# RazorClient/Stark-prover

Measured on AMD Instinct MI355X. Metric: FRI commit field-elems/sec at codeword 2^24; achieved HBM GB/s vs peak, higher is better.
Workload: dtype u32; 1 GPU; fri_commit codeword 2^24, blowup 8 (d=2^21), SHA-256 Merkle per layer, 21 rounds; codeword_log2=24, per_gpu_log2=24, blowup=8, field=p=3*2^30+1, parallelism=single GPU

## Files before the change

### stark-prover_amd/csrc/fri_commit.hip

```cpp
#include "fri_host.hpp"

void fri::plan_layout(Plan& p, size_t d, uint32_t log_n, uint32_t G, uint32_t rank, size_t& lay, size_t& tre,
                        size_t& xin) {
    const bool sharded = G > 1;
    uint32_t logG = 0;
    while ((1u << logG) < G) logG++;
    p.log_n = log_n;
    p.d = d;
    p.rmax = rounds_bound(d, log_n);
    p.sharded = sharded;
    p.G = G;
    p.rank = rank;
    p.k_sw = sharded ? switch_layer(log_n, logG, p.rmax) : -1;
    const bool local_tail = sharded && p.k_sw < p.rmax;
    p.cs0 = 0;
    if (sharded) {
        const size_t per = (d + G - 1) / G;
        while (((size_t)1 << p.cs0) < per) p.cs0++;
        if ((int)p.cs0 < p.k_sw) p.cs0 = (uint32_t)p.k_sw;
    }
    std::vector<uint32_t> block_of(G), rank_of(G);
    for (uint32_t r = 0; r < G; r++) block_of[r] = rank_of[r] = r;
    lay = tre = xin = 0;
    for (int k = 0; k <= p.rmax; k++) {
        const uint32_t L = log_n - (uint32_t)k;
        const bool blk = sharded && k <= p.k_sw;
        const uint32_t Lt = blk ? L - logG : L;
        p.layer_off[k] = lay;
        p.tree_off[k] = tre;
        p.xinv_off[k] = xin;
        p.xinv_start[k] = 0;
        p.block[k] = blk ? block_of[rank] : 0u;
        lay += (blk && !(k == p.k_sw && local_tail)) ? ((size_t)1 << Lt) : ((size_t)1 << L);
        tre += 8 * (((size_t)2 << Lt) - 1);
        if (k < p.rmax) {
            if (sharded && k < p.k_sw) {
                const size_t B = (size_t)1 << Lt;
                p.xinv_start[k] = fold_xinv_start(block_of[rank], G, B);
                xin += B / 2;
                advance_blocks(block_of, rank_of, G);
            } else {
                xin += ((size_t)1 << L) / 2;
            }
        }
    }
    p.layer_off[p.rmax + 1] = lay;
    p.tree_off[p.rmax + 1] = tre;
    p.xinv_off[p.rmax + 1] = xin;
}

int fri::plan_build(fri_ctx* ctx, size_t d, uint32_t log_n, uint32_t offset, uint32_t G, uint32_t rank) {
    Plan& p = ctx->plan;
    const bool sharded = G > 1;
    auto same = [&](const Plan& q) {
        return q.d == d && q.log_n == log_n && q.offset == offset && q.sharded == sharded && q.G == G && q.rank == rank;
    };
    if (p.valid && same(p)) return FRI_OK;
    bool stale = p.valid;
    for (const Lane& ln : ctx->lanes) stale = stale || (ln.plan.valid && !same(ln.plan));
    if (stale) plan_free(ctx);
    const size_t n = (size_t)1 << log_n;
    size_t lay, tre, xin;
    plan_layout(p, d, log_n, G, rank, lay, tre, xin);
    p.offset = offset;
    p.in_cap = d ? d : 1;
    p.coef_cap = d / 2 + 1;
    p.coefF_cap = 0;
    if (sharded) {
        const size_t S1 = p.cs0 >= 1 ? ((size_t)1 << (p.cs0 - 1)) : 1;
        const size_t Ssw = (size_t)1 << (p.cs0 - (uint32_t)p.k_sw);
        const bool local_tail = p.k_sw < p.rmax;
        p.coef_cap = std::max(S1, local_tail ? G * Ssw / 2 : (size_t)0) + 1;
        if (local_tail && p.k_sw >= 1) p.coefF_cap = G * Ssw;
    }
    const size_t nhi = log_n > POW_LO_LOG ? ((size_t)1 << (log_n - POW_LO_LOG)) : 1;
    if (dalloc(ctx, &p.d_in, p.in_cap * 4) != hipSuccess || dalloc(ctx, &p.coefA, p.coef_cap * 4) != hipSuccess ||
        dalloc(ctx, &p.coefB, p.coef_cap * 4) != hipSuccess ||
        (p.coefF_cap && dalloc(ctx, &p.coefF, p.coefF_cap * 4) != hipSuccess) ||
        dalloc(ctx, &p.layers, lay * 4) != hipSuccess ||
        dalloc(ctx, &p.trees, tre * 4) != hipSuccess || dalloc(ctx, &p.xinv, (xin ? xin : 1) * 4) != hipSuccess ||
        dalloc(ctx, &p.pre_lo, ((size_t)1 << POW_LO_LOG) * 4) != hipSuccess ||
        dalloc(ctx, &p.pre_hi, nhi * 4) != hipSuccess ||
        dalloc(ctx, &p.wgmax, 6 * ((log_n > 8 ? ((size_t)1 << (log_n - 8)) : 1) + 16) * 4) != hipSuccess) {
        plan_release(ctx, p);
        return fail(ctx, FRI_ENOMEM, "device allocation failed for commit plan");
    }
    hipStream_t s = ctx->stream;
    launch_pow_table(p.pre_lo, p.pre_hi, log_n, offset, 1u, s);
    if (sharded) {
        uint32_t offk = offset;
        for (int k = 0; k < p.rmax; k++) {
            const uint32_t L = log_n - (uint32_t)k;
            const size_t cnt = p.xinv_off[k + 1] - p.xinv_off[k];
            const uint32_t first = mul_std(offk, pow_std(root_of_unity(L), (uint64_t)p.xinv_start[k]));
            launch_coset_points(p.layers, cnt, first, L, s);
            launch_batch_inverse(p.layers, p.xinv + p.xinv_off[k], cnt, 1, s);
            offk = mul_std(offk, offk);
        }
    } else if (p.rmax > 0) {
        launch_coset_points(ctx->scratch_a, n / 2, offset, log_n, s);
        launch_batch_inverse(ctx->scratch_a, p.xinv + p.xinv_off[0], n / 2, 1, s);
        for (int k = 1; k < p.rmax; k++)
            launch_square_mont(p.xinv + p.xinv_off[k - 1], p.xinv + p.xinv_off[k], ((size_t)1 << (log_n - k)) / 2, s);
    }
    FRI_HIP(ctx, hipGetLastError());
    FRI_HIP(ctx, hipStreamSynchronize(s));
    p.valid = true;
    return FRI_OK;
}

uint32_t* fri::coef_buf(Plan& p, int r) {
    if (r == 0) return const_cast<uint32_t*>(p.src);
    return (r % 2 == 1) ? p.coefA : p.coefB;
}

LayerTask fri::commit_task(fri_ctx* ctx, int k) {
    Plan& p = ctx->plan;
    LayerTask t{};
    t.prev = k ? p.layers + p.layer_off[k - 1] : nullptr;
    t.xinv = k ? p.xinv + p.xinv_off[k - 1] : nullptr;
    t.values = p.layers + p.layer_off[k];
    t.tree = p.trees + p.tree_off[k];
    t.L = p.log_n - (uint32_t)k;
    t.k = k;
    t.coef_in = coef_buf(p, k ? k - 1 : 0);
    t.coef_out = k ? coef_buf(p, k) : nullptr;
    t.d0 = p.d;
    t.wgmax = p.wgmax;
    t.st = ctx->d_state;
    return t;
}

static void enqueue_commit(fri_ctx* ctx) {
    Plan& p = ctx->plan;
    hipStream_t s = ctx->stream;
    const uint32_t log_n = p.log_n;
    const size_t n = (size_t)1 << log_n;
    NttPlan np = lde_plan(ctx, log_n);
    np.pre_lo = p.pre_lo;
    np.pre_hi = p.pre_hi;
    np.scratch = p.trees;
    size_t sp = span_begin(ctx, "lde", p.d * 4 + n * 4);
    launch_ntt(np, p.src, p.d, p.layers + p.layer_off[0], s);
    span_end(ctx, sp);
    for (int k = 0; k <= p.rmax; k++) {
        const uint32_t L = log_n - (uint32_t)k;
        if (L <= TAIL_LOG) {
            LayerTask ts[TAIL_LOG + 1];
            uint32_t nt = 0;
            for (int kk = k; kk <= p.rmax; kk++) ts[nt++] = commit_task(ctx, kk);
            size_t spk = span_begin(ctx, k == 0 ? "layer0" : "layers", 0);
            launch_tail(ts, nt, s);
            span_end(ctx, spk);
            break;
        }
        const LayerTask t = commit_task(ctx, k);
        uint64_t leaf_nodes = 0;
        for (uint32_t j = 0; j <= 4 && j <= L; j++) leaf_nodes += (uint64_t)1 << (L - j);
        const uint64_t leaf_bytes = ((uint64_t)4 << L) + 4 * (uint64_t)p.d + 32 * leaf_nodes;
        size_t spl = (k == 0 && L >= 19) ? span_begin(ctx, "merkle_layer0_leaf", leaf_bytes) : (size_t)-1;
        size_t spk = span_begin(ctx, k == 0 ? "layer0" : "layers", 0);
        launch_layer(t, s, spl == (size_t)-1 ? nullptr : ctx->spans[spl].e);
        span_end(ctx, spk);
    }
}

void fri::init_state(fri_ctx* ctx, DevState* h, const fri_channel_state* chan_in, uint32_t flags,
                       const uint32_t* forced_betas) {
    ctx->h_state = h;
    ctx->res_lane = ctx->cur_lane;
    memset(h, 0, sizeof(DevState));
    ctx->commit_gen++;
    if (chan_in && chan_in->has_state) {
        for (int i = 0; i < 8; i++)
            h->chan[i] = ((uint32_t)chan_in->digest[4 * i] << 24) | ((uint32_t)chan_in->digest[4 * i + 1] << 16) |
                         ((uint32_t)chan_in->digest[4 * i + 2] << 8) | chan_in->digest[4 * i + 3];
        h->chan_has = 1;
    }
    h->deg0max = -1;
    h->final_degree = -1;
    for (int r = 0; r < MAXR; r++) { h->newmax[r] = -1; h->evenmax[r] = -1; h->oddmax[r] = -1; }
    for (int r = 0; r <= MAXR; r++) h->deg[r] = -1;
    if ((flags & FRI_FLAG_FORCE_BETAS) && forced_betas) {
        h->forced = 1;
        for (int r = 0; r < MAXR; r++) h->forced_beta[r] = forced_betas[r];
    }
}
int fri::commit_validate(fri_ctx* ctx, size_t d, uint32_t log_n, uint32_t offset, uint32_t flags,
                           const uint32_t* forced_betas) {
    if (log_n < 1 || log_n > ctx->log_n_max) return fail(ctx, FRI_EINVAL, "log_n out of range for context");
    const size_t n = (size_t)1 << log_n;
    if (d > n) return fail(ctx, FRI_EDEGREE, "more coefficients than domain points (domain would be exhausted)");
    if (offset == 0 || offset >= P) return fail(ctx, FRI_EINVAL, "offset must be a nonzero canonical element");
    if ((flags & FRI_FLAG_FORCE_BETAS) && !forced_betas) return fail(ctx, FRI_EINVAL, "forced betas missing");
    if (forced_betas && (flags & FRI_FLAG_FORCE_BETAS) && !check_canonical(forced_betas, MAXR))
        return fail(ctx, FRI_EINVAL, "forced beta not canonical");
    return FRI_OK;
}

int fri::commit_enqueue(fri_ctx* ctx, const uint32_t* host_coeffs, const uint32_t* dev_coeffs, size_t d,
                          uint32_t log_n, uint32_t offset, const fri_channel_state* chan_in, uint32_t flags,
                          const uint32_t* forced_betas, int slot) {
    int rv = commit_validate(ctx, d, log_n, offset, flags, forced_betas);
    if (rv) return rv;
    FRI_HIP(ctx, hipSetDevice(ctx->device));
    int rc = plan_build(ctx, d, log_n, offset);
    if (rc) return rc;
    Plan& p = ctx->plan;
    hipStream_t s = ctx->stream;
    ctx->sharded_layers = 0;
    DevState* hs = slot < 0 ? ctx->h_sync : ctx->h_slot[slot];
    init_state(ctx, hs, chan_in, flags, forced_betas);
    ctx->commit_log_n = log_n;
    if (dev_coeffs && d && ctx->user_in && dev_coeffs == ctx->user_in) {
        p.src = ctx->user_in;
    } else {
        if (host_coeffs && d)
            FRI_HIP(ctx, hipMemcpyAsync(p.d_in, host_coeffs, d * 4, hipMemcpyHostToDevice, s));
        else if (dev_coeffs && d && dev_coeffs != p.d_in)
            FRI_HIP(ctx, hipMemcpyAsync(p.d_in, dev_coeffs, d * 4, hipMemcpyDeviceToDevice, s));
        p.src = p.d_in;
    }
    const bool use_graph = !(flags & FRI_FLAG_NO_GRAPH) && !ctx->profiling;
    if (use_graph) {
        const int gs = slot < 0 ? FRI_MAX_INFLIGHT : slot;
        const int gv = p.src == p.d_in ? 0 : 1;
        hipGraph_t& pg = p.graph[gs][gv];
        hipGraphExec_t& px = p.exec[gs][gv];
        if (px && p.graph_src[gs][gv] != p.src) {
            FRI_HIP(ctx, hipStreamSynchronize(s));
            hipGraphExecDestroy(px);
            hipGraphDestroy(pg);
            px = nullptr;
            pg = nullptr;
        }
        if (!px) {
            FRI_HIP(ctx, hipStreamBeginCapture(s, hipStreamCaptureModeThreadLocal));
            hipError_t e1 = hipMemcpyAsync(ctx->d_state, hs, sizeof(DevState), hipMemcpyHostToDevice, s);
            if (e1 == hipSuccess) enqueue_commit(ctx);
            const hipError_t e2 =
                e1 == hipSuccess ? hipMemcpyAsync(hs, ctx->d_state, sizeof(DevState), hipMemcpyDeviceToHost, s) : e1;
            hipGraph_t g = nullptr;
            const hipError_t e3 = hipStreamEndCapture(s, &g);
            if (e2 != hipSuccess || e3 != hipSuccess) {
                if (g) hipGraphDestroy(g);
                FRI_HIP(ctx, e2);
                FRI_HIP(ctx, e3);
            }
            pg = g;
            FRI_HIP(ctx, hipGraphInstantiate(&px, g, nullptr, nullptr, 0));
            p.graph_src[gs][gv] = p.src;
        }
        FRI_HIP(ctx, hipGraphLaunch(px, s));
    } else {
        FRI_HIP(ctx, hipMemcpyAsync(ctx->d_state, hs, sizeof(DevState), hipMemcpyHostToDevice, s));
        enqueue_commit(ctx);
        FRI_HIP(ctx, hipGetLastError());
        FRI_HIP(ctx, hipMemcpyAsync(hs, ctx->d_state, sizeof(DevState), hipMemcpyDeviceToHost, s));
    }
    return FRI_OK;
}

int fri::commit_finish(fri_ctx* ctx, DevState* h, uint32_t log_n, fri_commit_result* out) {
    if (h->status) {
        h->n_layers = 0;
        return fail(ctx, (int)h->status, status_message(h->status));
    }
    memset(out, 0, sizeof *out);
    out->n_layers = h->n_layers;
    out->n_rounds = h->n_rounds;
    out->log_n = log_n;
    out->final_value = h->final_value;
    out->final_degree = h->final_degree;
    for (uint32_t k = 0; k < h->n_layers && k <= (uint32_t)MAXR; k++) digest_to_bytes(h->roots[k], out->roots[k]);
    for (uint32_t r = 0; r < h->n_rounds && r < (uint32_t)MAXR; r++) out->betas[r] = h->beta[r];
    digest_to_bytes(h->chan, out->channel_out.digest);
    out->channel_out.has_state = h->chan_has;
    ctx->err.clear();
    return FRI_OK;
}

int fri::run_commit(fri_ctx* ctx, const uint32_t* host_coeffs, const uint32_t* dev_coeffs, size_t d,
                      uint32_t log_n, uint32_t offset, const fri_channel_state* chan_in, uint32_t flags,
                      const uint32_t* forced_betas, fri_commit_result* out) {
    if (!ctx || !out) return fail(ctx, FRI_EINVAL, "null argument");
    int rc = commit_validate(ctx, d, log_n, offset, flags, forced_betas);
    if (rc) return rc;
    rc = use_lane(ctx, 0);
    if (rc) return rc;
    rc = commit_enqueue(ctx, host_coeffs, dev_coeffs, d, log_n, offset, chan_in, flags, forced_betas, -1);
    if (rc) return rc;
    FRI_HIP(ctx, hipStreamSynchronize(ctx->stream));
    ctx->async_unsettled = false;
    if (ctx->profiling) spans_collect(ctx);
    return commit_finish(ctx, ctx->h_state, log_n, out);
}

extern "C" int fri_commit(fri_ctx* ctx, const uint32_t* coeffs, size_t d, uint32_t log_n, uint32_t offset,
                          const fri_channel_state* chan_in, uint32_t flags, const uint32_t* forced_betas,
                          fri_commit_result* out) {
    if (d && !coeffs) return fail(ctx, FRI_EINVAL, "null coefficients");
    if (ctx && ctx->team_root) return team_commit(ctx, coeffs, nullptr, d, log_n, offset, chan_in, flags, forced_betas, out);
    return run_commit(ctx, coeffs, nullptr, d, log_n, offset, chan_in, flags, forced_betas, out);
}

extern "C" int fri_commit_device(fri_ctx* ctx, const uint32_t* d_coeffs, size_t d, uint32_t log_n,
                                 uint32_t offset, const fri_channel_state* chan_in, uint32_t flags,
                                 const uint32_t* forced_betas, fri_commit_result* out) {
    if (d && !d_coeffs) return fail(ctx, FRI_EINVAL, "null coefficients");
    if (ctx && ctx->team_root)
        return team_commit(ctx, nullptr, d_coeffs, d, log_n, offset, chan_in, flags, forced_betas, out);
    return run_commit(ctx, nullptr, d_coeffs, d, log_n, offset, chan_in, flags, forced_betas, out);
}
extern "C" int fri_debug_plan_layout(size_t d, uint32_t log_n, uint32_t world, uint32_t rank, uint64_t* out,
                                     size_t cap) {
    if (!out || log_n < 1 || log_n > 30 || world < 1 || world > 64 || (world & (world - 1)) || rank >= world)
        return FRI_EINVAL;
    uint32_t logG = 0;
    while ((1u << logG) < world) logG++;
    if (world > 1 && log_n < logG + 12) return FRI_EINVAL;
    if (cap < 4 + 5 * (size_t)(MAXR + 1)) return FRI_EINVAL;
    Plan p;
    size_t lay, tre, xin;
    plan_layout(p, d, log_n, world, rank, lay, tre, xin);
    out[0] = (uint64_t)p.rmax;
    out[1] = (uint64_t)(int64_t)p.k_sw;
    out[2] = 4 * (uint64_t)(lay + tre + xin);
    out[3] = p.cs0;
    for (int k = 0; k <= p.rmax; k++) {
        uint64_t* o = out + 4 + 5 * (size_t)k;
        o[0] = p.layer_off[k + 1] - p.layer_off[k];
        o[1] = p.tree_off[k + 1] - p.tree_off[k];
        o[2] = p.xinv_off[k + 1] - p.xinv_off[k];
        o[3] = p.xinv_start[k];
        o[4] = p.block[k];
    }
    return FRI_OK;
}
```

### stark-prover_amd/csrc/fri_host.hpp

```cpp
#pragma once
#include <hip/hip_runtime.h>
#include <stdio.h>
#include <string.h>
#include <algorithm>
#include <chrono>
#include <condition_variable>
#include <cstdlib>
#include <functional>
#include <map>
#include <memory>
#include <mutex>
#include <string>
#include <thread>
#include <vector>

#include <rccl/rccl.h>

#include "../../include/fri_amd.h"
#include "fri_internal.hpp"

#pragma GCC visibility push(hidden)

namespace fri {

static_assert(MAXR == FRI_MAX_ROUNDS, "round bound");

struct ProfEntry { double ms = 0; uint64_t launches = 0; uint64_t bytes = 0; };

struct Plan {
    bool valid = false;
    uint32_t log_n = 0;
    size_t d = 0;
    uint32_t offset = 0;
    int rmax = 0;
    bool sharded = false;
    uint32_t G = 1, rank = 0;
    int k_sw = -1;
    uint32_t cs0 = 0;
    uint32_t* coefF = nullptr;  size_t coefF_cap = 0;
    uint32_t* d_in = nullptr;   size_t in_cap = 0;
    const uint32_t* src = nullptr;
    uint32_t* coefA = nullptr;
    uint32_t* coefB = nullptr;  size_t coef_cap = 0;
    uint32_t* layers = nullptr; size_t layer_off[MAXR + 2] = {0};
    uint32_t* trees = nullptr;  size_t tree_off[MAXR + 2] = {0};
    uint32_t* xinv = nullptr;   size_t xinv_off[MAXR + 2] = {0};
    size_t xinv_start[MAXR + 2] = {0};
    uint32_t block[MAXR + 2] = {0};
    uint32_t* pre_lo = nullptr;
    uint32_t* pre_hi = nullptr;
    int32_t* wgmax = nullptr;
    hipGraph_t graph[FRI_MAX_INFLIGHT + 1][2] = {};
    hipGraphExec_t exec[FRI_MAX_INFLIGHT + 1][2] = {};
    const uint32_t* graph_src[FRI_MAX_INFLIGHT + 1][2] = {};
    hipGraph_t tail_graph = nullptr;
    hipGraphExec_t tail_exec = nullptr;
    const uint32_t* tail_src = nullptr;
    bool graph_profiled = false;
};

struct Lane {
    Plan plan;
    hipStream_t stream = nullptr;
    DevState* d_state = nullptr;
};

struct Team;

struct Transport {
    int rank = 0, world = 1;
    ncclComm_t comm = nullptr;
    ncclComm_t xcomm = nullptr;
    bool host = false;
    bool loop = false;
    bool peer = false;
    Team* team = nullptr;
    int64_t fail_at = -1;
    int64_t n_ops = 0;
    fri_collectives ops{};
    uint8_t* hs = nullptr;
    uint8_t* hr = nullptr;
    size_t hcap = 0;
    std::vector<fri_transport_op> log;
};

struct DistBuf {
    size_t cap = 0;
    uint32_t* cyc = nullptr;
    uint32_t* recv = nullptr;
    uint32_t* half = nullptr;
    uint32_t* half2 = nullptr;
    uint32_t* top = nullptr;
    uint32_t* pre_lo = nullptr;
    uint32_t* pre_hi = nullptr;
    size_t gcap = 0;
    uint32_t* gath = nullptr;
    uint32_t* dq = nullptr;
    uint32_t* rec = nullptr;
    ShardTop* shtop = nullptr;
    std::vector<ShardTop> shtop_h;
    std::vector<int32_t> sched_h;
};

struct PeerSlot {
    const void* send;
    void* recv;
    size_t bytes;
    uint32_t op, chan;
    int peer;
};

struct Team {
    uint32_t G = 1, logG = 0;
    int kind = FRI_TRANSPORT_PEER;
    std::vector<int> dev;
    std::vector<fri_ctx*> rk;
    bool can_pull = true;
    bool kernel_pull = true;
    std::vector<std::pair<int, int>> peer_pairs;
    std::vector<std::thread> th;
    std::mutex jm;
    std::condition_variable jcv, dcv;
    uint64_t seq = 0;
    uint32_t left = 0;
    bool quit = false;
    std::function<int(uint32_t)> job;
    std::vector<int> rc;
    std::mutex bm;
    std::condition_variable bcv;
    uint64_t bgen = 0;
    uint32_t arrived = 0;
    bool aborted = false;
    std::string why;
    std::vector<PeerSlot> slot;
    std::vector<hipEvent_t> ev_ready, ev_done;
};

struct TimedSpan { std::string cls; hipEvent_t b, e; uint64_t bytes; };
}

using namespace fri;

struct fri_ctx {
    int device = 0;
    uint32_t log_n_max = 0;
    hipStream_t stream = nullptr;
    std::string err;
    uint32_t* tw_fwd = nullptr;
    uint32_t* tw_inv = nullptr;
    uint32_t* scratch_a = nullptr;
    uint32_t* scratch_b = nullptr;
    uint32_t* scratch_c = nullptr;
    uint32_t* pow_lo = nullptr;
    uint32_t* pow_hi = nullptr;
    DevState* d_state = nullptr;
    DevState* h_state = nullptr;
    DevState* h_sync = nullptr;
    DevState* h_slot[FRI_MAX_INFLIGHT] = {};
    hipEvent_t ev_slot[FRI_MAX_INFLIGHT] = {};
    uint64_t slot_ticket[FRI_MAX_INFLIGHT] = {};
    uint32_t slot_log_n[FRI_MAX_INFLIGHT] = {};
    bool slot_pending[FRI_MAX_INFLIGHT] = {};
    bool slot_user[FRI_MAX_INFLIGHT] = {};
    uint32_t* h_in[FRI_MAX_INFLIGHT] = {};
    uint32_t* d_slot_in[FRI_MAX_INFLIGHT] = {};
    size_t h_in_cap[FRI_MAX_INFLIGHT] = {};
    hipEvent_t ev_in[FRI_MAX_INFLIGHT] = {};
    hipStream_t h2d_stream = nullptr;
    uint64_t next_ticket = 1;
    bool async_unsettled = false;
    Plan plan;
    Lane lanes[FRI_MAX_INFLIGHT];
    int cur_lane = 0;
    int res_lane = 0;
    int max_lanes = FRI_DEFAULT_LANES;
    int lanes_ok = FRI_MAX_INFLIGHT;
    int slot_lane[FRI_MAX_INFLIGHT] = {};
    uint64_t lane_ticket[FRI_MAX_INFLIGHT] = {};
    bool profiling = false;
    std::map<std::string, ProfEntry> prof;
    std::vector<TimedSpan> spans;
    std::vector<hipEvent_t> event_pool;
    size_t event_next = 0;
    Transport tp;
    DistBuf db;
    hipStream_t xstream = nullptr;
    hipEvent_t ev_vals = nullptr, ev_xchg = nullptr;
    hipStream_t cstream = nullptr;
    hipEvent_t ev_pre = nullptr, ev_coef = nullptr;
    uint32_t sharded_layers = 0;
    uint64_t commit_gen = 0;
    uint32_t commit_log_n = 0;
    uint32_t* interp_tmp = nullptr;
    size_t interp_cap = 0;
    uint32_t* dq_host = nullptr;
    uint32_t* dq_dev = nullptr;
    uint32_t* trace_tree = nullptr;
    uint32_t* trace_lde = nullptr;
    size_t trace_tree_cap = 0;
    bool trace_valid = false;
    uint32_t trace_log_t = 0, trace_log_b = 0, trace_offset = 0;
    bool stuck = false;
    bool inject_stall = false;
    uint32_t* stall_flag = nullptr;
    uint32_t* stall_flag_dev = nullptr;
    std::map<const void*, size_t> allocs;
    size_t dev_bytes = 0, dev_peak = 0;
    size_t dev_cap = 0;
    Team* team_root = nullptr;
    uint32_t* user_in = nullptr;
    size_t user_cap = 0;
    uint64_t* d_csum = nullptr;
    uint64_t* h_csum = nullptr;
};

namespace fri {

template <class T>
inline hipError_t dalloc(fri_ctx* ctx, T** p, size_t bytes) {
    void* q = nullptr;
    if (ctx->dev_cap && ctx->dev_bytes + bytes > ctx->dev_cap) { *p = nullptr; return hipErrorOutOfMemory; }
    const hipError_t e = hipMalloc(&q, bytes);
    if (e != hipSuccess) { *p = nullptr; return e; }
    *p = static_cast<T*>(q);
    ctx->allocs[q] = bytes;
    ctx->dev_bytes += bytes;
    if (ctx->dev_bytes > ctx->dev_peak) ctx->dev_peak = ctx->dev_bytes;
    return hipSuccess;
}
inline void dfree(fri_ctx* ctx, const void* p) {
    if (!p) return;
    auto it = ctx->allocs.find(p);
    if (it != ctx->allocs.end()) {
        ctx->dev_bytes -= it->second;
        ctx->allocs.erase(it);
    }
    hipFree(const_cast<void*>(p));
}

#define FRI_HIP(ctx, expr)                                                              \
    do {                                                                                \
        hipError_t _e = (expr);                                                         \
        if (_e != hipSuccess) {                                                         \
            (ctx)->err = std::string(#expr) + ": " + hipGetErrorString(_e);             \
            return FRI_EHIP;                                                            \
        }                                                                               \
    } while (0)

inline double rccl_timeout_s() {
    const char* e = getenv("FRI_RCCL_TIMEOUT_S");
    const double v = e ? atof(e) : 0.0;
    return v > 0.0 ? v : 120.0;
}
inline double seconds_since(std::chrono::steady_clock::time_point t0) {
    return std::chrono::duration<double>(std::chrono::steady_clock::now() - t0).count();
}
inline int fail(fri_ctx* ctx, int code, const std::string& msg) {
    if (ctx) ctx->err = msg;
    return code;
}

inline const char* status_message(uint32_t status) {
    return status == FRI_EINVAL ? "coefficient not canonical (>= p)"
                                : "degree exceeds the domain (reference would panic)";
}

inline bool check_canonical(const uint32_t* v, size_t n) {
    for (size_t i = 0; i < n; i += 16384) {
        const size_t e = n - i < 16384 ? n : i + 16384;
        uint32_t bad = 0;
        for (size_t j = i; j < e; j++) bad |= (uint32_t)(v[j] >= P);
        if (bad) return false;
    }
    return true;
}

inline int rounds_bound(size_t d, uint32_t log_n) {
    if (d <= 1) return 0;
    int b = 0;
    for (size_t v = d - 1; v; v >>= 1) b++;
    return b < (int)log_n ? b : (int)log_n;
}

constexpr uint32_t SHARD_MIN_LOG = 20;

inline bool next_layer_sharded(uint32_t log_n, uint32_t logG, int k, int rmax) {
    const uint32_t Lk = log_n - (uint32_t)k;
    return k < rmax && (Lk - 1) >= SHARD_MIN_LOG && (Lk - 1 - logG) >= 10;
}
inline int switch_layer(uint32_t log_n, uint32_t logG, int rmax) {
    int k = 0;
    while (next_layer_sharded(log_n, logG, k, rmax)) k++;
    return k;
}
inline void advance_blocks(std::vector<uint32_t>& block_of, std::vector<uint32_t>& rank_of, uint32_t G) {
    for (uint32_t r = 0; r < G; r++) {
        const uint32_t br = block_of[r];
        block_of[r] = br < G / 2 ? 2 * br : 2 * (br - G / 2) + 1;
    }
    for (uint32_t r = 0; r < G; r++) rank_of[block_of[r]] = r;
}
inline size_t fold_xinv_start(uint32_t b, uint32_t G, size_t B) {
    const bool isA = b < G / 2;
    return (size_t)(isA ? b : b - G / 2) * B + (isA ? 0 : B / 2);
}

inline NttPlan lde_plan(fri_ctx* ctx, uint32_t log_n) {
    NttPlan p{};
    p.log_n = log_n;
    p.tw = ctx->tw_fwd;
    return p;
}

inline int ensure_tmp(fri_ctx* ctx, size_t words) {
    if (words <= ctx->interp_cap) return FRI_OK;
    FRI_HIP(ctx, hipStreamSynchronize(ctx->stream));
    if (ctx->interp_tmp) dfree(ctx, ctx->interp_tmp);
    ctx->interp_tmp = nullptr;
    ctx->interp_cap = 0;
    if (dalloc(ctx, &ctx->interp_tmp, words * 4) != hipSuccess) return fail(ctx, FRI_ENOMEM, "partials scratch");
    ctx->interp_cap = words;
    return FRI_OK;
}
constexpr size_t TMP_KEEP_WORDS = (size_t)1 << 26;
inline void tmp_trim(fri_ctx* ctx) {
    if (ctx->interp_cap <= TMP_KEEP_WORDS) return;
    (void)hipStreamSynchronize(ctx->stream);
    dfree(ctx, ctx->interp_tmp);
    ctx->interp_tmp = nullptr;
    ctx->interp_cap = 0;
}

inline void digest_to_bytes(const uint32_t* w, uint8_t* out) {
    for (int i = 0; i < 8; i++) {
        out[4 * i] = (uint8_t)(w[i] >> 24); out[4 * i + 1] = (uint8_t)(w[i] >> 16);
        out[4 * i + 2] = (uint8_t)(w[i] >> 8); out[4 * i + 3] = (uint8_t)w[i];
    }
}

size_t span_begin(fri_ctx* ctx, const char* cls, uint64_t bytes);
void span_end(fri_ctx* ctx, size_t id);
void spans_collect(fri_ctx* ctx);

void plan_release(fri_ctx* ctx, Plan& p);
void plan_free(fri_ctx* ctx);
int use_lane(fri_ctx* ctx, int j);
void settle(fri_ctx* ctx);

void plan_layout(Plan& p, size_t d, uint32_t log_n, uint32_t G, uint32_t rank, size_t& lay, size_t& tre,
                 size_t& xin);
int plan_build(fri_ctx* ctx, size_t d, uint32_t log_n, uint32_t offset, uint32_t G = 1, uint32_t rank = 0);
uint32_t* coef_buf(Plan& p, int r);
LayerTask commit_task(fri_ctx* ctx, int k);
void init_state(fri_ctx* ctx, DevState* h, const fri_channel_state* chan_in, uint32_t flags,
                const uint32_t* forced_betas);
int commit_validate(fri_ctx* ctx, size_t d, uint32_t log_n, uint32_t offset, uint32_t flags,
                    const uint32_t* forced_betas);
int commit_enqueue(fri_ctx* ctx, const uint32_t* host_coeffs, const uint32_t* dev_coeffs, size_t d,
                   uint32_t log_n, uint32_t offset, const fri_channel_state* chan_in, uint32_t flags,
                   const uint32_t* forced_betas, int slot);
int commit_finish(fri_ctx* ctx, DevState* h, uint32_t log_n, fri_commit_result* out);
int run_commit(fri_ctx* ctx, const uint32_t* host_coeffs, const uint32_t* dev_coeffs, size_t d, uint32_t log_n,
               uint32_t offset, const fri_channel_state* chan_in, uint32_t flags, const uint32_t* forced_betas,
               fri_commit_result* out);

int dq_alloc(fri_ctx* ctx);

int input_checksum(fri_ctx* ctx, const uint32_t* d_src, size_t d, uint64_t* out);

int tp_host_stage(fri_ctx* ctx, size_t bytes);
void rccl_abort(fri_ctx* ctx);
int sync_sharded(fri_ctx* ctx, hipStream_t s);
int tp_allgather(fri_ctx* ctx, const void* dsend, void* drecv, size_t bytes, hipStream_t s);
int tp_alltoall(fri_ctx* ctx, const void* dsend, void* drecv, size_t bytes_per_peer, hipStream_t s);
int tp_sendrecv(fri_ctx* ctx, const void* dsend, void* drecv, size_t bytes, int peer, hipStream_t s, uint32_t chan);
int dist_buffers(fri_ctx* ctx, size_t M, uint32_t G, size_t gwords);

int run_commit_sharded(fri_ctx* ctx, const uint32_t* host_coeffs, const uint32_t* dev_coeffs, size_t d,
                       uint32_t log_n, uint32_t offset, const fri_channel_state* chan_in, uint32_t flags,
                       const uint32_t* forced_betas, fri_commit_result* out);
int decommit_sharded(fri_ctx* ctx, uint64_t index, uint32_t* values, size_t values_cap, uint8_t* paths,
                     size_t paths_cap, size_t* paths_len);

void team_abort(Team* T, const std::string& why);
bool team_barrier(Team* T);
int team_run(fri_ctx* root, const std::function<int(uint32_t)>& fn);
void team_destroy(fri_ctx* root);
int team_commit(fri_ctx* ctx, const uint32_t* host_coeffs, const uint32_t* dev_coeffs, size_t d, uint32_t log_n,
                uint32_t offset, const fri_channel_state* chan_in, uint32_t flags, const uint32_t* forced_betas,
                fri_commit_result* out);
int team_layer_copy(fri_ctx* ctx, uint32_t layer, uint32_t* out);
int team_tree_level_copy(fri_ctx* ctx, uint32_t layer, uint32_t level, uint32_t* w);
int team_decommit(fri_ctx* ctx, uint64_t index, uint32_t* values, size_t values_cap, uint8_t* paths,
                  size_t paths_cap, size_t* paths_len);

}

#pragma GCC visibility pop
```

### stark-prover_amd/csrc/fri_internal.hpp

```cpp
#pragma once
#include <hip/hip_runtime.h>
#include <stddef.h>
#include <stdint.h>
#include <functional>
#include "field.hpp"

namespace fri {

constexpr int MAXR = 32;
constexpr uint32_t TOP_LOG = 9;
#ifndef FRI_TAIL_LOG
#define FRI_TAIL_LOG 9
#endif
constexpr uint32_t TAIL_LOG = FRI_TAIL_LOG;
constexpr uint32_t POW_LO_LOG = 12;

struct DevState {
    uint32_t chan[8];
    uint32_t chan_has;
    uint32_t chan_pending;
    uint32_t n_layers;
    uint32_t n_rounds;
    uint32_t final_value;
    int32_t  final_degree;
    uint32_t status;
    uint32_t forced;
    int32_t  deg0max;
    uint32_t active[MAXR + 1];
    int32_t  deg[MAXR + 1];
    int32_t  newmax[MAXR];
    int32_t  evenmax[MAXR];
    int32_t  oddmax[MAXR];
    uint32_t beta[MAXR];
    uint32_t beta_mont[MAXR];
    uint32_t forced_beta[MAXR];
    uint32_t roots[MAXR + 1][8];
#ifdef FRI_STAMPS
    uint64_t stamps[MAXR + 1][64];
#endif
};

__host__ __device__ inline size_t level_offset(uint32_t L, uint32_t l) {
    return ((size_t)2 << L) - ((size_t)2 << (L - l));
}

struct NttPlan {
    uint32_t log_n;
    const uint32_t* tw;
    const uint32_t* pre_lo;
    const uint32_t* pre_hi;
    const uint32_t* post_lo;
    const uint32_t* post_hi;
    uint32_t* scratch;
};
void launch_ntt(const NttPlan& p, const uint32_t* src, size_t d, uint32_t* dst, hipStream_t s);

void launch_twiddles(uint32_t* tw, uint32_t log_max, bool inverse, hipStream_t s);
void launch_pow_table(uint32_t* lo, uint32_t* hi, uint32_t log_n, uint32_t base_std,
                      uint32_t scale_std, hipStream_t s);
void launch_batch_inverse(const uint32_t* in, uint32_t* out, size_t n, int out_mont,
                          hipStream_t s);
void launch_coset_points(uint32_t* out, size_t count, uint32_t offset, uint32_t log_n,
                         hipStream_t s);
void launch_square_mont(const uint32_t* in, uint32_t* out, size_t count, hipStream_t s);
size_t interp_tmp_words(size_t n, uint32_t log_N);
void launch_interp_weights(const uint32_t* xs, size_t n, uint32_t* acc, uint32_t* tmp, hipStream_t s);
void launch_interp_coeffs(const uint32_t* ys, uint32_t* w_to_c, size_t n, hipStream_t s);
void launch_interp_eval(const uint32_t* xs, const uint32_t* c, size_t n, uint32_t log_N, uint32_t* f, uint32_t* tmp,
                        hipStream_t s);
size_t evaluate_tmp_words(size_t d, size_t count);
void launch_evaluate(const uint32_t* coeffs, size_t d, const uint32_t* xs, size_t count, uint32_t* out,
                     uint32_t* tmp, hipStream_t s);
void launch_poly_pointwise_mul(const uint32_t* a, const uint32_t* b, uint32_t* out, size_t n, hipStream_t s);
void launch_poly_newton(const uint32_t* f, const uint32_t* g, uint32_t* out, size_t n, hipStream_t s);
constexpr size_t POLY_DIRECT_LIMIT = 4096;
void launch_poly_conv_direct(const uint32_t* lng, size_t ll, const uint32_t* sht, size_t ls, uint32_t* out,
                             size_t n_out, hipStream_t s);
void launch_poly_reverse(const uint32_t* src, size_t top, size_t cnt, uint32_t* dst, size_t n, hipStream_t s);
void launch_poly_sub(const uint32_t* a, const uint32_t* t, uint32_t* r, size_t n, hipStream_t s);
struct DecommitPlan {
    uint64_t index;
    uint32_t log_n, n_layers;
    uint64_t layer_off[MAXR + 1];
    uint64_t tree_off[MAXR + 1];
    uint32_t path_off[MAXR + 1];
    uint32_t logG;
    uint8_t shard_lb1[MAXR + 1];
    uint8_t val_block[MAXR + 1];
    uint64_t owned[MAXR + 1];
    uint64_t top_off[MAXR + 1];
};
void launch_decommit_gather(const uint32_t* layers, const uint32_t* trees, const DecommitPlan& dp, uint32_t* out,
                            hipStream_t s, const uint32_t* top = nullptr);
void launch_fold_plain(const uint32_t* in, uint32_t* out, uint32_t log_m, const uint32_t* xinv_m,
                       uint32_t beta, hipStream_t s);

constexpr uint32_t REC_WORDS = 16;
struct ShardTop {
    uint32_t* rec_out;
    const int32_t* rec_mx;
    const uint32_t* rec_c0;
    uint32_t rec_R;
    uint32_t G;
    const uint32_t* recs_in;
    int32_t sched_deg;
    uint32_t sched_on;
    uint8_t rank_of_block[64];
};

struct LayerTask {
    const uint32_t* prev;
    const uint32_t* xinv;
    uint32_t* values;
    uint32_t* tree;
    uint32_t L;
    int k;
    uint32_t beta_m;
    const uint32_t* coef_in;
    uint32_t* coef_out;
    size_t d0;
    int32_t* wgmax;
    DevState* st;
    const DevState* gst;
    int gidx;
    size_t jlo, jhi, ibase, obase;
    const ShardTop* shard;
    const uint32_t* prev2;
    uint32_t send_half;
    uint32_t wg_base;
    uint32_t wg_total;
};
void launch_layer(const LayerTask& t, hipStream_t s, hipEvent_t ev_leaf_end = nullptr,
                  const std::function<void()>& after_leaf = {}, hipEvent_t ev_before_top = nullptr,
                  const std::function<void()>& after_part1 = {});
void launch_tail(const LayerTask* ts, uint32_t n, hipStream_t s);
void launch_coef(const LayerTask& t, uint32_t G, hipStream_t s);
void launch_coset_coeffs(const uint32_t* a, size_t d, uint32_t* out, size_t M, uint32_t c_std, hipStream_t s);
void launch_decimate(const uint32_t* a, size_t d, uint32_t* ev, uint32_t* od, hipStream_t s);
void launch_radix2_block(const uint32_t* E, const uint32_t* O, const uint32_t* tlo, const uint32_t* thi,
                         uint32_t* out, size_t M, uint32_t negate, hipStream_t s);
void launch_cyclic_to_block(const uint32_t* recv, uint32_t* block, size_t B, uint32_t G, hipStream_t s);
void launch_place_blocks(const uint32_t* gath, uint32_t* layer, size_t B, uint32_t G, const uint32_t* block_of,
                         hipStream_t s);
struct PeerPull {
    const uint32_t* src[64];
    uint32_t* dst;
    size_t words;
    uint32_t n;
    uint32_t vec4;
};
void launch_peer_pull(const PeerPull& pp, hipStream_t s);
void launch_checksum(const uint32_t* v, size_t n, uint64_t* out, hipStream_t s);
void launch_replicate(const uint32_t* src, uint32_t* dst, size_t words, uint32_t G, hipStream_t s);
void launch_top(const LayerTask& t, uint32_t l, const int32_t* mx, uint32_t G, hipStream_t s);

constexpr uint32_t FIBSQ_MAX_B = 16;
struct FibsqParams {
    uint32_t log_n;
    uint32_t B;
    uint32_t offset_m;
    uint32_t w_m, winv_m;
    uint32_t glast_m, gprev_m;
    uint32_t a_last;
    uint32_t alpha_m[3];
    uint32_t zinv_m[FIBSQ_MAX_B];
};
void launch_fibsq_cp(const uint32_t* f_lde, uint32_t* out, const FibsqParams& q, hipStream_t s);
void launch_trace_gather(const uint32_t* lde, const uint32_t* tree, uint32_t L, uint64_t index, uint64_t stride,
                         uint32_t count, uint32_t* out, hipStream_t s);

}
```

### stark-prover_amd/csrc/fri_layer.hip

```cpp
#include "fri_internal.hpp"
#include "sha256_fast.hpp"
#include "sha256_quad.hpp"

namespace fri {

constexpr uint32_t INV2_M2 = 0x80000000u;

#ifdef FRI_STAMPS
#define TOP_STAMP(i)                                                                     \
    do {                                                                                 \
        if (COMMIT && threadIdx.x == 0) t.st->stamps[t.k][(i)] = __builtin_amdgcn_s_memrealtime(); \
    } while (0)
#define TOP_CLK(i)                                                                               \
    do {                                                                                           \
        if (COMMIT && threadIdx.x == 0) t.st->stamps[t.k][(i)] = __builtin_amdgcn_s_memtime();     \
    } while (0)
#define TOP_STAMP_T(i, tid_)                                                                       \
    do {                                                                                           \
        if (COMMIT && threadIdx.x == (tid_)) t.st->stamps[t.k][(i)] = __builtin_amdgcn_s_memrealtime(); \
    } while (0)
#else
#define TOP_STAMP(i) do {} while (0)
#define TOP_CLK(i) do {} while (0)
#define TOP_STAMP_T(i, tid_) do {} while (0)
#endif
#ifdef FRI_STAMPS
#define WIDE_STAMP(i)                                                                              \
    do {                                                                                           \
        if (COMMIT && blockIdx.x == 0 && threadIdx.x == 0) t.st->stamps[t.k][(i)] = __builtin_amdgcn_s_memrealtime(); \
    } while (0)
#else
#define WIDE_STAMP(i) do {} while (0)
#endif
#ifdef FRI_STAMPS
#define TAIL_STAMP_T(i, tid_, fn)                                                  \
    do {                                                                           \
        if (threadIdx.x == (tid_)) t.st->stamps[t.k][(i)] = fn();                  \
    } while (0)
#define TAIL_STAMP(i) TAIL_STAMP_T(i, 0, __builtin_amdgcn_s_memrealtime)
#define TAIL_CLK(i) TAIL_STAMP_T(i, 0, __builtin_amdgcn_s_memtime)
#else
#define TAIL_STAMP_T(i, tid_, fn) do {} while (0)
#define TAIL_STAMP(i) do {} while (0)
#define TAIL_CLK(i) do {} while (0)
#endif

__device__ __forceinline__ uint32_t fold1(uint32_t a, uint32_t b, uint32_t xinv_m, uint32_t beta_m) {
    uint32_t s = add(a, b), t = sub(a, b);
    return mmul(add(s, mmul(mmul(t, xinv_m), beta_m)), INV2_M2);
}

#ifndef FRI_CHAIN_PRIO
#define FRI_CHAIN_PRIO 3
#endif
__device__ __forceinline__ void chain_prio() {
    if (FRI_CHAIN_PRIO > 0) __builtin_amdgcn_s_setprio(FRI_CHAIN_PRIO);
}

struct Dg { uint32_t w[8]; };

__device__ __forceinline__ void dg_load(const uint32_t* p, Dg& d) {
    uint4 a = reinterpret_cast<const uint4*>(p)[0], b = reinterpret_cast<const uint4*>(p)[1];
    d.w[0] = a.x; d.w[1] = a.y; d.w[2] = a.z; d.w[3] = a.w; d.w[4] = b.x; d.w[5] = b.y; d.w[6] = b.z; d.w[7] = b.w;
}
__device__ __forceinline__ void dg_store(uint32_t* p, const Dg& d) {
    reinterpret_cast<uint4*>(p)[0] = make_uint4(d.w[0], d.w[1], d.w[2], d.w[3]);
    reinterpret_cast<uint4*>(p)[1] = make_uint4(d.w[4], d.w[5], d.w[6], d.w[7]);
}
__device__ __forceinline__ void dg_lds_load(const uint4* p, Dg& d) {
    uint4 a = p[0], b = p[1];
    d.w[0] = a.x; d.w[1] = a.y; d.w[2] = a.z; d.w[3] = a.w; d.w[4] = b.x; d.w[5] = b.y; d.w[6] = b.z; d.w[7] = b.w;
}
__device__ __forceinline__ void dg_lds_store(uint4* p, const Dg& d) {
    p[0] = make_uint4(d.w[0], d.w[1], d.w[2], d.w[3]);
    p[1] = make_uint4(d.w[4], d.w[5], d.w[6], d.w[7]);
}
__device__ __forceinline__ void hnode(const Dg& l, const Dg& r, Dg& o) { shaf::node(l.w, r.w, o.w); }
__device__ __forceinline__ void hleaf(uint32_t v, Dg& o) { shaf::leaf(v, o.w); }
__device__ __forceinline__ void cnode(const Dg& l, const Dg& r, Dg& o) { shaf::node_compact(l.w, r.w, o.w); }
__device__ __forceinline__ void cleaf(uint32_t v, Dg& o) { shaf::leaf_compact(v, o.w); }

__device__ __forceinline__ void pair_level(const uint4* A, uint4* B, uint32_t* out, uint32_t tid, uint32_t cnt,
                                           const shaq::Role& R) {
    if (tid >= max(2 * cnt, 64u)) return;
    const uint32_t q = (tid >> 1) & (cnt - 1), half = (tid & 1u) ^ 1u;
    const bool real = tid < 2 * cnt;
    Dg a, b;
    dg_lds_load(A + 4 * q, a);
    dg_lds_load(A + 4 * q + 2, b);
    uint32_t o[4];
    shaq::node(a.w, b.w, o, R);
    if (!real) return;
    const uint4 v = make_uint4(o[0], o[1], o[2], o[3]);
    B[2 * q + half] = v;
    reinterpret_cast<uint4*>(out + 8 * q)[half] = v;
}

#ifndef FRI_SCHED_PRODUCER
#define FRI_SCHED_PRODUCER 1
#endif
#ifndef FRI_SCHED_CHANNEL
#define FRI_SCHED_CHANNEL 0
#endif
struct SchedLds {
    uint32_t wk[32 * 48];
    uint32_t flag;
};
__device__ __forceinline__ void sched_init(SchedLds* sl) {
    if (FRI_SCHED_PRODUCER && threadIdx.x == 0) sl->flag = 0u;
}
__device__ __forceinline__ void pair_level_s(const uint4* A, uint4* B, uint32_t* out, uint32_t tid, uint32_t cnt,
                                             const shaq::Role& R, SchedLds* sl, uint32_t ord) {
    if (!FRI_SCHED_PRODUCER || cnt > 32) {
        pair_level(A, B, out, tid, cnt, R);
        return;
    }
    const uint32_t wv = tid >> 6;
    if (wv > 1) return;
    const uint32_t lane = tid & 63u;
    const uint32_t q = (lane >> 1) & (cnt - 1), half = (lane & 1u) ^ 1u;
    const bool real = lane < 2 * cnt;
    Dg a, b;
    dg_lds_load(A + 4 * q, a);
    dg_lds_load(A + 4 * q + 2, b);
    if (wv == 1) {
        uint32_t w[16];
#pragma unroll
        for (int i = 0; i < 8; i++) { w[i] = a.w[i]; w[8 + i] = b.w[i]; }
        shaq::produce(w, sl->wk + 48 * q, &sl->flag, 3u * ord, real && (lane & 1u) == 0u, lane == 0u, R);
        return;
    }
    uint32_t o[4];
    shaq::node_ext(a.w, b.w, o, R, sl->wk + 48 * q, &sl->flag, 3u * ord);
    if (!real) return;
    const uint4 v = make_uint4(o[0], o[1], o[2], o[3]);
    B[2 * q + half] = v;
    reinterpret_cast<uint4*>(out + 8 * q)[half] = v;
}

__device__ __forceinline__ void lds_barrier() {
    asm volatile("s_waitcnt lgkmcnt(0)\n\ts_barrier" ::: "memory");
}

__device__ __forceinline__ int wave_max_i(int v) {
#pragma unroll
    for (int off = 32; off > 0; off >>= 1) v = max(v, __shfl_xor(v, off));
    return v;
}

__device__ __forceinline__ void coef_slice(const LayerTask& t, uint32_t w, uint32_t G, int32_t* red, uint32_t t0,
                                           uint32_t nthr) {
    int m0 = -1, m1 = -1, m2 = -1;
    const uint32_t tx = threadIdx.x - t0;
    const size_t jhi_all = t.jhi ? t.jhi : ~(size_t)0;
    if (t.k == 0) {
        const size_t a = t.jlo, b = min(t.d0, jhi_all), n = b > a ? b - a : 0;
        const size_t cs = (n + G - 1) / G, lo = a + (size_t)w * cs, hi = min(b, lo + cs);
        const uint32_t* in = t.coef_in - t.ibase;
        for (size_t j = lo + tx; j < hi; j += nthr) {
            const uint32_t c = in[j];
            if (c) m0 = max(m0, (int)j);
            if (c >= P) m1 = 0;
        }
    } else {
        const DevState* st = t.st;
        const size_t len = (size_t)(st->deg[t.k - 1] + 1), nlen = (len + 1) / 2;
        const uint32_t beta_m = st->beta_mont[t.k - 1];
        const size_t a = t.jlo, b = min(nlen, jhi_all), n = b > a ? b - a : 0;
        const size_t cs = (n + G - 1) / G, lo = a + (size_t)w * cs, hi = min(b, lo + cs);
        const uint32_t* in = t.coef_in - t.ibase;
        uint32_t* outp = t.coef_out - t.obase;
        for (size_t j = lo + tx; j < hi; j += nthr) {
            uint32_t e = in[2 * j];
            uint32_t o = (2 * j + 1 < len) ? in[2 * j + 1] : 0u;
            uint32_t v = add(e, mmul(o, beta_m));
            outp[j] = v;
            if (v) m0 = (int)j;
            if (e) m1 = (int)j;
            if (o) m2 = (int)j;
        }
    }
    m0 = wave_max_i(m0); m1 = wave_max_i(m1); m2 = wave_max_i(m2);
    const uint32_t wave = tx >> 6;
    if ((tx & 63) == 0) { red[3 * wave] = m0; red[3 * wave + 1] = m1; red[3 * wave + 2] = m2; }
}
__device__ __forceinline__ void coef_combine(const LayerTask& t, uint32_t w, const int32_t* red, uint32_t nw) {
    int a = -1, b = -1, c = -1;
    for (uint32_t i = 0; i < nw; i++) { a = max(a, red[3 * i]); b = max(b, red[3 * i + 1]); c = max(c, red[3 * i + 2]); }
    t.wgmax[3 * w] = a; t.wgmax[3 * w + 1] = b; t.wgmax[3 * w + 2] = c;
}
__device__ __forceinline__ void coef_task(const LayerTask& t, uint32_t w, uint32_t G, int32_t* red ) {
    coef_slice(t, w, G, red, 0, blockDim.x);
    lds_barrier();
    if (threadIdx.x == 0) coef_combine(t, w, red, blockDim.x / 64);
}

#ifndef FRI_QUAD_LEAVES_FIRST
#define FRI_QUAD_LEAVES_FIRST 1
#endif
template <bool LEAVES>
__device__ __forceinline__ void quad(const uint4& vals, const uint32_t* in0, uint32_t* lv0, uint32_t* lv1,
                                     size_t q , Dg& out) {
    Dg a, b, n0, n1;
#if FRI_QUAD_LEAVES_FIRST
    if (LEAVES) {
        Dg c, d;
        hleaf(vals.x, a); hleaf(vals.y, b); hleaf(vals.z, c); hleaf(vals.w, d);
        dg_store(lv0 + 8 * (4 * q), a); dg_store(lv0 + 8 * (4 * q + 1), b);
        dg_store(lv0 + 8 * (4 * q + 2), c); dg_store(lv0 + 8 * (4 * q + 3), d);
        hnode(a, b, n0);
        hnode(c, d, n1);
        dg_store(lv1 + 8 * (2 * q), n0);
        dg_store(lv1 + 8 * (2 * q + 1), n1);
        hnode(n0, n1, out);
        return;
    }
#endif
    if (LEAVES) { hleaf(vals.x, a); hleaf(vals.y, b); dg_store(lv0 + 8 * (4 * q), a); dg_store(lv0 + 8 * (4 * q + 1), b); }
    else { dg_load(in0 + 8 * (4 * q), a); dg_load(in0 + 8 * (4 * q + 1), b); }
    hnode(a, b, n0);
    dg_store(lv1 + 8 * (2 * q), n0);
    if (LEAVES) { hleaf(vals.z, a); hleaf(vals.w, b); dg_store(lv0 + 8 * (4 * q + 2), a); dg_store(lv0 + 8 * (4 * q + 3), b); }
    else { dg_load(in0 + 8 * (4 * q + 2), a); dg_load(in0 + 8 * (4 * q + 3), b); }
    hnode(a, b, n1);
    dg_store(lv1 + 8 * (2 * q + 1), n1);
    hnode(n0, n1, out);
}

template <uint32_t TPB>
__device__ __forceinline__ void lds_two_levels(uint4* lds, const Dg& mine, uint32_t* lv2, uint32_t* lv3, uint32_t* lv4,
                                               size_t g2 ) {
    uint4* A = lds;
    uint4* B = lds + 2 * TPB;
    const uint32_t t = threadIdx.x;
    dg_store(lv2 + 8 * (g2 + t), mine);
    dg_lds_store(A + 2 * t, mine);
    lds_barrier();
    if (t < TPB / 2) {
        Dg l, r, o;
        dg_lds_load(A + 4 * t, l); dg_lds_load(A + 4 * t + 2, r);
        hnode(l, r, o);
        dg_lds_store(B + 2 * t, o);
        dg_store(lv3 + 8 * (g2 / 2 + t), o);
    }
    lds_barrier();
    if (t < TPB / 4) {
        Dg l, r, o;
        dg_lds_load(B + 4 * t, l); dg_lds_load(B + 4 * t + 2, r);
        hnode(l, r, o);
        dg_store(lv4 + 8 * (g2 / 4 + t), o);
    }
}

__device__ __forceinline__ bool gated_off(const LayerTask& t) {
    return t.gst && t.gidx >= 0 && !t.gst->active[t.gidx];
}

__device__ __forceinline__ uint32_t pair_beta(const LayerTask& t) { return t.gst->beta_mont[t.gidx]; }

template <bool FOLD, bool COMMIT, uint32_t TPB, bool PAIR = false>
__global__ __launch_bounds__(TPB) void k_layer_leaf(LayerTask t) {
    if (gated_off(t)) return;
    __shared__ uint4 lds[3 * TPB];
    __shared__ int32_t red[3 * (TPB / 64)];
    const uint32_t L = t.L;
    const size_t wg = PAIR ? (size_t)blockIdx.x + t.wg_base : (size_t)blockIdx.x;
    const size_t q = wg * TPB + threadIdx.x;
    uint4 v;
    if (FOLD) {
        const size_t half = (size_t)1 << L;
        const uint32_t beta_m = COMMIT ? t.st->beta_mont[t.k - 1] : (PAIR ? pair_beta(t) : t.beta_m);
        uint4 a = reinterpret_cast<const uint4*>(t.prev)[q];
        uint4 b = reinterpret_cast<const uint4*>(PAIR ? t.prev2 : t.prev + half)[q];
        uint4 x = reinterpret_cast<const uint4*>(t.xinv)[q];
        v.x = fold1(a.x, b.x, x.x, beta_m); v.y = fold1(a.y, b.y, x.y, beta_m);
        v.z = fold1(a.z, b.z, x.z, beta_m); v.w = fold1(a.w, b.w, x.w, beta_m);
        reinterpret_cast<uint4*>(t.values)[q] = v;
    } else {
        v = reinterpret_cast<const uint4*>(t.values)[q];
    }
    uint32_t* tr = t.tree;
    Dg top;
    quad<true>(v, nullptr, tr + 8 * level_offset(L, 0), tr + 8 * level_offset(L, 1), q, top);
    if (COMMIT) coef_task(t, blockIdx.x, gridDim.x, red);
    lds_two_levels<TPB>(lds, top, tr + 8 * level_offset(L, 2), tr + 8 * level_offset(L, 3),
                        tr + 8 * level_offset(L, 4), wg * TPB);
}

#ifndef WIDE_PAIR_MAX
#define WIDE_PAIR_MAX (1u << 16)
#endif

__host__ __device__ __forceinline__ uint32_t wide_levels(uint32_t L) { return L <= 8 + TOP_LOG ? 8u : 4u; }

template <bool FOLD, bool COMMIT, bool PAIR = false>
__global__ __launch_bounds__(256) void k_layer_leaf_wide(LayerTask t) {
    if (gated_off(t)) return;
    WIDE_STAMP(60);
    __shared__ uint4 lds[2 * 256 + 2 * 128];
    __shared__ int32_t red[12];
    __shared__ SchedLds sl;
    sched_init(&sl);
    const uint32_t L = t.L;
    const size_t wg = PAIR ? (size_t)blockIdx.x + t.wg_base : (size_t)blockIdx.x;
    const size_t grid = PAIR ? (size_t)t.wg_total : (size_t)gridDim.x;
    const size_t i = wg * 256 + threadIdx.x;
    uint32_t v;
    if (FOLD) {
        const size_t half = (size_t)1 << L;
        const uint32_t beta_m = COMMIT ? t.st->beta_mont[t.k - 1] : (PAIR ? pair_beta(t) : t.beta_m);
        v = fold1(t.prev[i], PAIR ? t.prev2[i] : t.prev[i + half], t.xinv[i], beta_m);
        t.values[i] = v;
    } else {
        v = t.values[i];
    }
    uint32_t* tr = t.tree;
    Dg d;
    cleaf(v, d);
    dg_store(tr + 8 * i, d);
    uint4* A = lds;
    uint4* B = lds + 2 * 256;
    dg_lds_store(A + 2 * threadIdx.x, d);
    lds_barrier();
    WIDE_STAMP(61);
    uint32_t cnt = 256;
    const shaq::Role qr = shaq::role_of(threadIdx.x);
    if (grid * 128 < WIDE_PAIR_MAX) chain_prio();
    const uint32_t nlev = wide_levels(L);
#pragma unroll 1
    for (uint32_t j = 1; j <= nlev; j++) {
        cnt >>= 1;
        uint32_t* out = tr + 8 * (level_offset(L, j) + (wg << (8 - j)));
        if ((size_t)cnt * grid < WIDE_PAIR_MAX) {
            pair_level_s(A, B, out, threadIdx.x, cnt, qr, &sl, j);
        } else if (threadIdx.x < cnt) {
            Dg a, b, o;
            dg_lds_load(A + 4 * threadIdx.x, a);
            dg_lds_load(A + 4 * threadIdx.x + 2, b);
            hnode(a, b, o);
            dg_lds_store(B + 2 * threadIdx.x, o);
            dg_store(out + 8 * threadIdx.x, o);
        }
        if (COMMIT && j == 2 && threadIdx.x >= 128) coef_slice(t, blockIdx.x, gridDim.x, red, 128, 128);
        lds_barrier();
        uint4* tmp = A; A = B; B = tmp;
    }
    if (COMMIT && threadIdx.x == 128) coef_combine(t, blockIdx.x, red, 2);
    WIDE_STAMP(62);
}

__device__ __forceinline__ void reduce_mx(const int32_t* in, int32_t* out, uint32_t w, uint32_t R) {
    if (threadIdx.x >= 64) return;
    const uint32_t i = R * w + threadIdx.x;
    int a = -1, b = -1, c = -1;
    if (threadIdx.x < R) { a = in[3 * i]; b = in[3 * i + 1]; c = in[3 * i + 2]; }
    a = wave_max_i(a); b = wave_max_i(b); c = wave_max_i(c);
    if (threadIdx.x == 0) { out[3 * w] = a; out[3 * w + 1] = b; out[3 * w + 2] = c; }
}

#ifndef MID_PAIR_BY_WG
#define MID_PAIR_BY_WG 0
#endif

template <uint32_t NIN>
__global__ __launch_bounds__(NIN / 2) void k_tree_mid(uint32_t* tree, uint32_t L, uint32_t l, const DevState* st,
                                                      int gate, const int32_t* mx_in, int32_t* mx_out, uint32_t R) {
    if (st && gate >= 0 && !st->active[gate]) return;
    if (NIN == 256) chain_prio();
    __shared__ uint4 lds[NIN + NIN / 2];
    __shared__ SchedLds sl;
    sched_init(&sl);
    uint4* A = lds;
    uint4* B = lds + NIN;
    const uint32_t t = threadIdx.x;
    const size_t base = (size_t)blockIdx.x * NIN;
    const uint32_t* in = tree + 8 * level_offset(L, l);
    {
        Dg a, b, o;
        dg_load(in + 8 * (base + 2 * t), a);
        dg_load(in + 8 * (base + 2 * t + 1), b);
        if (mx_in) reduce_mx(mx_in, mx_out, blockIdx.x, R);
        hnode(a, b, o);
        dg_lds_store(A + 2 * t, o);
        dg_store(tree + 8 * (level_offset(L, l + 1) + (base >> 1) + t), o);
    }
    lds_barrier();
    const shaq::Role qr = shaq::role_of(t);
    uint32_t cnt = NIN / 2;
#pragma unroll 1
    for (uint32_t j = 2; j <= 4; j++) {
        cnt >>= 1;
        uint32_t* out = tree + 8 * (level_offset(L, l + j) + (base >> j));
        const bool narrow = NIN == 1024 && !MID_PAIR_BY_WG ? (size_t)cnt * gridDim.x < WIDE_PAIR_MAX
                                                           : 2 * cnt <= NIN / 2;
        if (narrow) {
            pair_level_s(A, B, out, t, cnt, qr, &sl, j);
        } else if (t < cnt) {
            Dg a, b, o;
            dg_lds_load(A + 4 * t, a);
            dg_lds_load(A + 4 * t + 2, b);
            hnode(a, b, o);
            dg_lds_store(B + 2 * t, o);
            dg_store(out + 8 * t, o);
        }
        lds_barrier();
        uint4* tmp = A; A = B; B = tmp;
    }
}

__global__ __launch_bounds__(256) void k_tree_mid8(uint32_t* tree, uint32_t L, uint32_t l, const DevState* st,
                                                   int gate, const int32_t* mx_in, int32_t* mx_out, uint32_t R) {
    if (st && gate >= 0 && !st->active[gate]) return;
    chain_prio();
    __shared__ uint4 lds[256 + 128];
    __shared__ SchedLds sl;
    sched_init(&sl);
    uint4* A = lds;
    uint4* B = lds + 256;
    const uint32_t t = threadIdx.x;
    const size_t base = (size_t)blockIdx.x * 256;
    const uint32_t* in = tree + 8 * level_offset(L, l);
    const shaq::Role qr = shaq::role_of(t);
    {
        const uint32_t q = t >> 1, half = (t & 1u) ^ 1u;
        Dg a, b;
        dg_load(in + 8 * (base + 2 * q), a);
        dg_load(in + 8 * (base + 2 * q + 1), b);
        if (mx_in) reduce_mx(mx_in, mx_out, blockIdx.x, R);
        uint32_t o[4];
        shaq::node(a.w, b.w, o, qr);
        const uint4 v = make_uint4(o[0], o[1], o[2], o[3]);
        A[2 * q + half] = v;
        reinterpret_cast<uint4*>(tree + 8 * (level_offset(L, l + 1) + (base >> 1) + q))[half] = v;
    }
    lds_barrier();
    uint32_t cnt = 128;
#pragma unroll 1
    for (uint32_t j = 2; j <= 8; j++) {
        cnt >>= 1;
        pair_level_s(A, B, tree + 8 * (level_offset(L, l + j) + (base >> j)), t, cnt, qr, &sl, j);
        lds_barrier();
        uint4* tmp = A; A = B; B = tmp;
    }
}

__device__ __forceinline__ void ktouch(const void* sym) {
    uint32_t a, b, c, d;
    asm volatile("s_nop 4\n\t"
                 "s_load_dword %0, %4, 0x0\n\ts_load_dword %1, %4, 0x40\n\t"
                 "s_load_dword %2, %4, 0x80\n\ts_load_dword %3, %4, 0xc0\n\t"
                 "s_waitcnt lgkmcnt(0)"
                 : "=&s"(a), "=&s"(b), "=&s"(c), "=&s"(d)
                 : "s"(sym)
                 : "memory");
}
__device__ __forceinline__ void kcache_touch_sha_tables() {
    ktouch(&shaf::KTAB[0]);
    ktouch(&shaf::PAD_KW_C.kw[0]);
    ktouch(&shaf::PAD_KW_1024.kw[0]);
    ktouch(&shaf::PAD_KW_1536.kw[0]);
}

__device__ __forceinline__ uint32_t hexch(uint32_t nib) { return nib < 10u ? 0x30u + nib : 0x57u + nib; }
__device__ __forceinline__ void hex2(uint32_t x, uint32_t& hi, uint32_t& lo) {
    hi = (hexch(x >> 28) << 24) | (hexch((x >> 24) & 15u) << 16) | (hexch((x >> 20) & 15u) << 8) | hexch((x >> 16) & 15u);
    lo = (hexch((x >> 12) & 15u) << 24) | (hexch((x >> 8) & 15u) << 16) | (hexch((x >> 4) & 15u) << 8) | hexch(x & 15u);
}
__device__ __forceinline__ uint32_t hexhex(uint32_t b) {
    const uint32_t x = ((b & 0xF0u) << 12) | (b & 0x0Fu);
    const uint32_t ge = ((x + 0x00060006u) >> 4) & 0x00010001u;
    return 0x33303330u + x + ge * 0x2F7u;
}

enum { CJ_REHASH = 0, CJ_MID = 2, CJ_ROOT = 3, CJ_FINAL = 6, CJ_END_ROUND = 6, CJ_END_FINAL = 8 };

__device__ __forceinline__ void chan_job(int j, uint32_t cs[8], uint32_t X[4], uint32_t has, const uint4* root_lds,
                                         uint32_t fv, const shaq::Role& R, const uint32_t* wk = nullptr,
                                         const uint32_t* flag = nullptr, uint32_t base = 0) {
    j = __builtin_amdgcn_readfirstlane(j);
    has = __builtin_amdgcn_readfirstlane(has);
    uint32_t w[16];
    const bool pad = (j == 1) || (j == 5);
    if (j == 0 || j == 2 || j == 6) {
#pragma unroll
        for (int i = 0; i < 8; i++) hex2(cs[i], w[2 * i], w[2 * i + 1]);
#pragma unroll
        for (int i = 0; i < 4; i++) X[i] = R.iv[i];
    } else if (j == 3 || j == 4) {
        const uint32_t b = (__lane_id() & 15u) + (j == 4 ? 16u : 0u);
        const uint32_t rw = reinterpret_cast<const uint32_t*>(root_lds)[b >> 2];
        const uint32_t hh = hexhex((rw >> (24 - 8 * (b & 3))) & 255u);
#pragma unroll
        for (int jj = 0; jj < 16; jj++) w[jj] = __builtin_amdgcn_readlane(hh, jj);
        if (j == 3 && !has) {
#pragma unroll
            for (int i = 0; i < 4; i++) X[i] = R.iv[i];
        }
    } else if (j == 7) {
#pragma unroll
        for (int i = 0; i < 16; i++) w[i] = 0u;
        w[0] = 0x30303030u; w[1] = 0x30303030u;
        hex2(fv, w[2], w[3]);
        w[4] = 0x80000000u;
        w[15] = 80u * 8u;
    }
    if (pad) shaq::compress_kw(X, j == 1 ? shaf::PAD_KW_C.kw : (has ? shaf::PAD_KW_1536.kw : shaf::PAD_KW_1024.kw), R);
    else if (wk && (j == 3 || j == 4)) shaq::compress_ext(X, w, R, wk + 48 * (j - 3), flag, base + 3 * (j - 3));
    else shaq::compress(X, w, R);
    if (j == 1 || j == 5 || j == 7) {
#pragma unroll
        for (int i = 0; i < 4; i++) {
            const uint32_t o = shaq::swap01(X[i]);
            cs[i] = R.is_a ? X[i] : o;
            cs[4 + i] = R.is_a ? o : X[i];
        }
    }
}

__device__ __forceinline__ void chan_produce(const uint4* root_lds, SchedLds* sl, uint32_t base, const shaq::Role& R) {
    const uint32_t lane = __lane_id();
#pragma unroll 1
    for (uint32_t jb = 0; jb < 2; jb++) {
        const uint32_t b = (lane & 15u) + 16u * jb;
        const uint32_t rw = reinterpret_cast<const uint32_t*>(root_lds)[b >> 2];
        const uint32_t hh = hexhex((rw >> (24 - 8 * (b & 3))) & 255u);
        uint32_t w[16];
#pragma unroll
        for (int jj = 0; jj < 16; jj++) w[jj] = __builtin_amdgcn_readlane(hh, jj);
        shaq::produce(w, sl->wk + 48 * jb, &sl->flag, base + 3 * jb, lane == 0, lane == 0, R);
    }
}

constexpr uint32_t pow2_32k_mod_p(int k) {
    uint64_t r = 1;
    for (int j = 0; j < k; j++) r = (r << 32) % P;
    return (uint32_t)r;
}
__device__ __forceinline__ uint32_t chan_beta(const uint32_t s[8]) {
    constexpr uint32_t W[8] = {pow2_32k_mod_p(8), pow2_32k_mod_p(7), pow2_32k_mod_p(6), pow2_32k_mod_p(5),
                               pow2_32k_mod_p(4), pow2_32k_mod_p(3), pow2_32k_mod_p(2), pow2_32k_mod_p(1)};
    uint32_t t[8];
#pragma unroll
    for (int i = 0; i < 8; i++) t[i] = mmul(s[i] >= P ? s[i] - P : s[i], W[i]);
    return add(add(add(t[0], t[1]), add(t[2], t[3])), add(add(t[4], t[5]), add(t[6], t[7])));
}

template <bool FROM_LEAVES, bool FOLD, bool COMMIT, bool SHARD = false>
__global__ __launch_bounds__(512) void k_tree_top(LayerTask t, uint32_t l, const int32_t* mx, uint32_t G) {
    if (gated_off(t)) return;
    chain_prio();
    __shared__ uint4 lds[2 * 1024 + 2 * 512];
    __shared__ int32_t red[24];
    __shared__ SchedLds sl;
    sched_init(&sl);
    const uint32_t L = t.L;
    const uint32_t N = 1u << (L - l);
    const uint32_t tid = threadIdx.x;

    const bool chan_wave = COMMIT && tid >= 448;
    DevState* st = t.st;
    uint32_t cs[8], X[4];
    uint32_t has = 0, forced = 0, fbeta = 0;
    int job = CJ_END_FINAL;
    if (chan_wave) {
#pragma unroll
        for (int i = 0; i < 8; i++) cs[i] = st->chan[i];
        const uint32_t h = st->chan_has, pend = st->chan_pending;
        const uint32_t fo = COMMIT ? st->forced : 0u, fb = st->forced_beta[t.k < MAXR ? t.k : 0];
        has = h;
        job = !h ? CJ_ROOT : (pend ? CJ_REHASH : CJ_MID);
        forced = fo;
        if (fo && t.k < MAXR) fbeta = fb;
    }
    if (tid >= 384 && tid < 448) kcache_touch_sha_tables();
    uint4* A = lds;
    uint4* B = lds + 2 * 1024;
    uint32_t* tr = t.tree;
    TOP_STAMP(0);
    if (FROM_LEAVES) {
        const size_t half = (size_t)1 << L;
        const uint32_t beta_m = FOLD ? (COMMIT ? st->beta_mont[t.k - 1] : t.beta_m) : 0u;
        for (uint32_t i = tid; i < max(N, 64u); i += blockDim.x) {
            const uint32_t j = i & (N - 1);
            const bool real = i < N;
            uint32_t v;
            if (FOLD) {
                v = fold1(t.prev[j], t.prev[j + half], t.xinv[j], beta_m);
                if (real) t.values[j] = v;
            } else {
                v = t.values[j];
            }
            Dg d;
            cleaf(v, d);
            if (real) {
                dg_store(tr + 8 * j, d);
                dg_lds_store(A + 2 * j, d);
            }
        }
        if (COMMIT) coef_task(t, 0, 1, red);
    } else if (SHARD && COMMIT) {
        const ShardTop& sh = *t.shard;
        for (uint32_t i = tid; i < N; i += blockDim.x) {
            Dg d;
            dg_load(sh.recs_in + REC_WORDS * sh.rank_of_block[i], d);
            dg_lds_store(A + 2 * i, d);
            dg_store(tr + 8 * i, d);
        }
        int m0 = -1, m1 = -1, m2 = -1;
        if (tid < sh.G) {
            const int32_t* rm = reinterpret_cast<const int32_t*>(sh.recs_in + REC_WORDS * tid + 8);
            m0 = rm[0]; m1 = rm[1]; m2 = rm[2];
            if (sh.sched_on) { m0 = sh.sched_deg; m1 = t.k == 0 ? -1 : 0; m2 = -1; }
        }
        m0 = wave_max_i(m0); m1 = wave_max_i(m1); m2 = wave_max_i(m2);
        if ((tid & 63) == 0) { red[3 * (tid >> 6)] = m0; red[3 * (tid >> 6) + 1] = m1; red[3 * (tid >> 6) + 2] = m2; }
    } else {
        const uint32_t* in = tr + 8 * level_offset(L, l);
        int p0 = -1, p1 = -1, p2 = -1;
        if (COMMIT && tid < G) { p0 = mx[3 * tid]; p1 = mx[3 * tid + 1]; p2 = mx[3 * tid + 2]; }
        for (uint32_t i = tid; i < N; i += blockDim.x) {
            Dg d;
            dg_load(in + 8 * i, d);
            dg_lds_store(A + 2 * i, d);
        }
        if (SHARD && !COMMIT) {
            const ShardTop& sh = *t.shard;
            int m0 = -1, m1 = -1, m2 = -1;
            for (uint32_t i = tid; i < sh.rec_R; i += blockDim.x) {
                m0 = max(m0, sh.rec_mx[3 * i]); m1 = max(m1, sh.rec_mx[3 * i + 1]); m2 = max(m2, sh.rec_mx[3 * i + 2]);
            }
            m0 = wave_max_i(m0); m1 = wave_max_i(m1); m2 = wave_max_i(m2);
            if ((tid & 63) == 0) { red[3 * (tid >> 6)] = m0; red[3 * (tid >> 6) + 1] = m1; red[3 * (tid >> 6) + 2] = m2; }
        }
        if (COMMIT) {
            int m0 = p0, m1 = p1, m2 = p2;
            for (uint32_t i = tid + blockDim.x; i < G; i += blockDim.x) {
                m0 = max(m0, mx[3 * i]); m1 = max(m1, mx[3 * i + 1]); m2 = max(m2, mx[3 * i + 2]);
            }
            m0 = wave_max_i(m0); m1 = wave_max_i(m1); m2 = wave_max_i(m2);
            if ((tid & 63) == 0) { red[3 * (tid >> 6)] = m0; red[3 * (tid >> 6) + 1] = m1; red[3 * (tid >> 6) + 2] = m2; }
        }
    }
    lds_barrier();
    int deg = -1;
    bool noncanon = false;
    if (COMMIT) {
        int m0 = -1, m1 = -1, m2 = -1;
#pragma unroll
        for (int i = 0; i < 8; i++) { m0 = max(m0, red[3 * i]); m1 = max(m1, red[3 * i + 1]); m2 = max(m2, red[3 * i + 2]); }
        deg = (t.k == 0) ? m0 : (m1 < 0 ? m2 : m0);
        noncanon = t.k == 0 && m1 >= 0;
    }
    const bool is_final = COMMIT && deg < 1;
    const int job_end = is_final ? CJ_END_FINAL : CJ_END_ROUND;
    uint32_t fv = 0;
    if (chan_wave && is_final && deg == 0)
        fv = SHARD ? t.shard->recs_in[11] : (t.k == 0 ? t.coef_in : t.coef_out)[0];
    TOP_STAMP(1);
    TOP_CLK(17);
    const uint32_t nlev = L - l;
    const uint32_t total = nlev + (COMMIT ? 1u : 0u);
    const uint32_t it_root = COMMIT ? nlev : ~0u;
    const bool chan_prod = FRI_SCHED_CHANNEL && COMMIT && tid >= 384 && tid < 448;
    const shaq::Role R = shaq::role_of(tid);
    uint32_t cnt = N;
#pragma unroll 1
    for (uint32_t it = 0; it < total; it++) {
        const bool level = it < nlev;
        if (level) {
            cnt >>= 1;
            uint32_t* out = tr + 8 * level_offset(L, l + 1 + it);
            if (cnt <= 128) {
#ifdef FRI_STAMPS
                if (it < 18 && tid == 0) TOP_CLK(24 + 2 * it);
#endif
                pair_level_s(A, B, out, tid, cnt, R, &sl, it);
#ifdef FRI_STAMPS
                if (it < 18 && tid == 0) TOP_CLK(25 + 2 * it);
#endif
            } else {
#pragma unroll 1
                for (uint32_t q = tid; q < cnt; q += blockDim.x) {
                    Dg a, b, o;
                    dg_lds_load(A + 4 * q, a);
                    dg_lds_load(A + 4 * q + 2, b);
#ifdef FRI_STAMPS
                    if (it < 18 && q == 0) { asm volatile("s_waitcnt lgkmcnt(0)" ::: "memory"); TOP_CLK(24 + 2 * it); }
#endif
                    cnode(a, b, o);
#ifdef FRI_STAMPS
                    if (it < 18 && q == 0) TOP_CLK(25 + 2 * it);
#endif
                    dg_lds_store(B + 2 * q, o);
                    dg_store(out + 8 * q, o);
                }
            }
        }
        if (chan_wave && job < job_end && (level ? (cnt <= 192 && job < CJ_ROOT) : true)) {
            do {
#ifdef FRI_STAMPS
                if (job == CJ_ROOT) TOP_STAMP_T(14, 448);
                if (job == CJ_ROOT + 2) TOP_STAMP_T(13, 448);
#endif
                chan_job(job, cs, X, has, A, fv, R, FRI_SCHED_CHANNEL ? sl.wk : nullptr, &sl.flag, 3u * it_root);
#ifdef FRI_STAMPS
                if (job >= CJ_ROOT && job <= CJ_ROOT + 2) TOP_STAMP_T(20 + job - CJ_ROOT, 448);
#endif
                job++;
            } while (!level && job < job_end);
        }
        if (chan_prod && it == it_root) chan_produce(A, &sl, 3u * it_root, R);
        lds_barrier();
        if (level) {
            uint4* tmp = A; A = B; B = tmp;
            if (it < 11) TOP_STAMP(2 + it);
            if (it + 1 == nlev) { TOP_CLK(18); TOP_STAMP(19); }
        }
    }
    if (SHARD && !COMMIT && tid == 448) {
        const ShardTop& sh = *t.shard;
        int m0 = -1, m1 = -1, m2 = -1;
#pragma unroll
        for (int i = 0; i < 8; i++) { m0 = max(m0, red[3 * i]); m1 = max(m1, red[3 * i + 1]); m2 = max(m2, red[3 * i + 2]); }
        Dg root;
        dg_lds_load(A, root);
        uint32_t* rec = sh.rec_out;
        dg_store(rec, root);
        reinterpret_cast<uint4*>(rec)[2] = make_uint4((uint32_t)m0, (uint32_t)m1, (uint32_t)m2, sh.rec_c0[0]);
        reinterpret_cast<uint4*>(rec)[3] = make_uint4(0u, 0u, 0u, 0u);
    }
    if (!COMMIT || tid != 448) return;
    const int k = t.k;
    if (noncanon) {
        st->active[k] = 0;
        st->status = 1u;
        return;
    }
    st->deg[k] = deg;
    Dg root;
    dg_lds_load(A, root);
#pragma unroll
    for (int i = 0; i < 8; i++) st->roots[k][i] = root.w[i];
    st->n_layers = (uint32_t)k + 1;
    TOP_STAMP_T(15, 448);
    if (deg >= 1 && k < MAXR && L >= 1) {
        uint32_t beta = chan_beta(cs);
#pragma unroll
        for (int i = 0; i < 8; i++) st->chan[i] = cs[i];
        st->chan_has = 1;
        st->chan_pending = 1;
        if (forced) beta = fbeta;
        st->beta[k] = beta;
        st->beta_mont[k] = to_mont(beta);
        st->active[k] = 1;
        st->n_rounds = (uint32_t)k + 1;
        TOP_STAMP_T(16, 448);
    } else {
        st->active[k] = 0;
        if (deg >= 1) { st->status = 7u; return; }
#pragma unroll
        for (int i = 0; i < 8; i++) st->chan[i] = cs[i];
        st->final_value = fv;
        st->final_degree = deg;
        st->chan_has = 1;
        st->chan_pending = 0;
    }
}

struct TailTask {
    LayerTask t[TAIL_LOG + 1];
    uint32_t n;
};

template <bool FOLD0>
__global__ __launch_bounds__(512) void k_tree_tail(TailTask tt) {
    const LayerTask& t0 = tt.t[0];
    if (gated_off(t0)) return;
    chain_prio();
    constexpr uint32_t NMAX = 1u << TAIL_LOG;
    __shared__ uint4 lds[2 * NMAX + NMAX];
    __shared__ uint32_t vals[2][NMAX];
    __shared__ uint32_t coefs[2][NMAX];
    __shared__ int32_t red[24];
    __shared__ uint32_t s_beta_m, s_active;
    __shared__ int32_t s_deg;
    __shared__ uint32_t s_fbeta[TAIL_LOG + 2];
    __shared__ uint32_t xv[2 * NMAX];
    __shared__ SchedLds sl;
    sched_init(&sl);
    uint32_t ord = 0;
    const uint32_t tid = threadIdx.x;
    const bool chan_wave = tid >= 448;
    DevState* st = t0.st;
    auto prefetch_x = [&](uint32_t t0p, uint32_t nthr) {
        uint32_t off = 1u << tt.t[0].L;
        for (uint32_t li = 1; li < tt.n; li++) {
            const uint32_t N = 1u << tt.t[li].L;
            for (uint32_t j = tid - t0p; j < N; j += nthr) xv[off + j] = tt.t[li].xinv[j];
            off += N;
        }
    };
    uint32_t cs[8], X[4];
    uint32_t has = 0;
    if (chan_wave) {
#pragma unroll
        for (int i = 0; i < 8; i++) cs[i] = st->chan[i];
        has = st->chan_has;
    }
    uint32_t pending = chan_wave ? st->chan_pending : 0u;
    if (tid >= 384 && tid < 448) kcache_touch_sha_tables();
    if (tid < tt.n + 1) {
        const int kk = t0.k + (int)tid;
        s_fbeta[tid] = (st->forced && kk < MAXR) ? st->forced_beta[kk] + 1u : 0u;
    }
    uint32_t beta_m = FOLD0 ? st->beta_mont[t0.k - 1] : 0u;
    int prev_deg = FOLD0 ? st->deg[t0.k - 1] : -1;
    const shaq::Role R = shaq::role_of(tid);
    uint32_t xoff = 0;
#pragma unroll 1
    for (uint32_t li = 0; li < tt.n; li++) {
        const LayerTask& t = tt.t[li];
        const int k = t.k;
        const uint32_t L = t.L, N = 1u << L;
        const uint32_t* xl = li ? xv + xoff : t.xinv;
        xoff += N;
        const bool fold = FOLD0 || li > 0;
        uint32_t* cur_v = vals[li & 1];
        const uint32_t* prev_v = vals[(li & 1) ^ 1];
        uint32_t* cur_c = coefs[li & 1];
        const uint32_t* prev_c = coefs[(li & 1) ^ 1];
        uint4* A = lds;
        uint4* B = lds + 2 * NMAX;
        uint32_t* tr = t.tree;
        TAIL_STAMP(0);
        for (uint32_t i = tid; i < max(N, 64u); i += blockDim.x) {
            const uint32_t j = i & (N - 1);
            const bool real = i < N;
            uint32_t v;
            if (fold) {
                const uint32_t a = li ? prev_v[j] : t.prev[j], b = li ? prev_v[j + N] : t.prev[j + N];
                v = fold1(a, b, xl[j], beta_m);
                if (real) t.values[j] = v;
            } else {
                v = t.values[j];
            }
            if (real) cur_v[j] = v;
            Dg d;
            cleaf(v, d);
            if (real) {
                dg_store(tr + 8 * j, d);
                dg_lds_store(A + 2 * j, d);
            }
        }
        const uint32_t nlev = L;
        const uint32_t coef_it = N > 256 ? 1u : 0u;
        const bool coef_late = nlev > coef_it;
        auto coef_fold = [&](uint32_t t0c, uint32_t nthr) {
            int m0 = -1, m1 = -1, m2 = -1;
            const uint32_t tx = tid - t0c;
            if (k == 0) {
                for (size_t j = tx; j < t.d0; j += nthr) {
                    const uint32_t c = t.coef_in[j];
                    if (c) m0 = max(m0, (int)j);
                    if (c >= P) m1 = 0;
                }
            } else {
                const uint32_t len = (uint32_t)(prev_deg + 1), nlen = (len + 1) / 2;
                const bool in_lds = li > 0 && k >= 2;
                for (uint32_t j = tx; j < nlen; j += nthr) {
                    const uint32_t e = in_lds ? prev_c[2 * j] : t.coef_in[2 * j];
                    const uint32_t o = (2 * j + 1 < len) ? (in_lds ? prev_c[2 * j + 1] : t.coef_in[2 * j + 1]) : 0u;
                    const uint32_t v = add(e, mmul(o, beta_m));
                    cur_c[j] = v;
                    if (v) m0 = (int)j;
                    if (e) m1 = (int)j;
                    if (o) m2 = (int)j;
                }
            }
            m0 = wave_max_i(m0); m1 = wave_max_i(m1); m2 = wave_max_i(m2);
            const uint32_t w = tx >> 6;
            if ((tx & 63) == 0) { red[3 * w] = m0; red[3 * w + 1] = m1; red[3 * w + 2] = m2; }
        };
        if (!coef_late) coef_fold(0, blockDim.x);
        if (li == 0 && !coef_late) prefetch_x(0, blockDim.x);
        lds_barrier();
        TAIL_STAMP(1);
        TAIL_CLK(17);
        int deg = 1;
        bool noncanon = false;
        int job_end = CJ_END_ROUND;
        uint32_t fv = 0;
        auto settle = [&](uint32_t nw) {
            int a = -1, b = -1, c = -1;
            for (uint32_t i = 0; i < nw; i++) { a = max(a, red[3 * i]); b = max(b, red[3 * i + 1]); c = max(c, red[3 * i + 2]); }
            deg = (k == 0) ? a : (b < 0 ? c : a);
            noncanon = k == 0 && b >= 0;
            job_end = deg < 1 ? CJ_END_FINAL : CJ_END_ROUND;
            if (chan_wave && deg == 0) fv = (k == 0) ? t.coef_in[0] : cur_c[0];
        };
        if (!coef_late) settle(8);
        int job = CJ_END_FINAL;
        if (chan_wave) job = !has ? CJ_ROOT : (pending ? CJ_REHASH : CJ_MID);
        const uint32_t total = nlev + 1;
        const uint32_t it_root = nlev;
        uint32_t ch_base = 0;
        uint32_t cnt = N;
#pragma unroll 1
        for (uint32_t it = 0; it < total; it++) {
            const bool level = it < nlev;
            if (level) {
                cnt >>= 1;
                uint32_t* out = tr + 8 * level_offset(L, 1 + it);
                if (cnt <= 128) {
                    if (it < 18) TAIL_CLK(24 + 2 * it);
                    pair_level_s(A, B, out, tid, cnt, R, &sl, ord++);
                    if (it < 18) TAIL_CLK(25 + 2 * it);
                } else {
#pragma unroll 1
                    for (uint32_t q = tid; q < cnt; q += blockDim.x) {
                        Dg a, b, o;
                        dg_lds_load(A + 4 * q, a);
                        dg_lds_load(A + 4 * q + 2, b);
                        cnode(a, b, o);
                        dg_lds_store(B + 2 * q, o);
                        dg_store(out + 8 * q, o);
                    }
                }
            }
            if (!level && it == it_root) ch_base = 3u * (ord++), ord++;
            if (chan_wave && job < job_end && (level ? (cnt <= 192 && job < CJ_ROOT) : true)) {
                do {
                    chan_job(job, cs, X, has, A, fv, R, FRI_SCHED_CHANNEL ? sl.wk : nullptr, &sl.flag, ch_base);
#ifdef FRI_STAMPS
                    if (job >= CJ_ROOT && job <= CJ_ROOT + 2) TAIL_STAMP_T(20 + job - CJ_ROOT, 448, __builtin_amdgcn_s_memrealtime);
#endif
                    job++;
                } while (!level && job < job_end);
            }
            if (FRI_SCHED_CHANNEL && tid >= 384 && tid < 448 && !level && it == it_root) chan_produce(A, &sl, ch_base, R);
            if (coef_late && it == coef_it && tid >= 256 && tid < 384) coef_fold(256, 128);
            if (li == 0 && coef_late && it == coef_it && tid >= 384 && tid < 448) prefetch_x(384, 64);
            lds_barrier();
            if (coef_late && it == coef_it) settle(2);
            if (level) {
                uint4* tmp = A; A = B; B = tmp;
                if (it < 11) TAIL_STAMP(2 + it);
                if (it + 1 == nlev) { TAIL_CLK(18); TAIL_STAMP(19); }
            }
        }
        if (tid == 448 && noncanon) {
            st->active[k] = 0;
            st->status = 1u;
            s_active = 0;
        } else if (tid == 448) {
            st->deg[k] = deg;
            Dg root;
            dg_lds_load(A, root);
#pragma unroll
            for (int i = 0; i < 8; i++) st->roots[k][i] = root.w[i];
            st->n_layers = (uint32_t)k + 1;
            uint32_t active = 0, bm = 0;
            if (deg >= 1 && k < MAXR && L >= 1) {
                uint32_t beta = chan_beta(cs);
#pragma unroll
                for (int i = 0; i < 8; i++) st->chan[i] = cs[i];
                st->chan_has = 1;
                st->chan_pending = 1;
                if (s_fbeta[li]) beta = s_fbeta[li] - 1u;
                st->beta[k] = beta;
                bm = to_mont(beta);
                st->beta_mont[k] = bm;
                st->active[k] = 1;
                st->n_rounds = (uint32_t)k + 1;
                active = 1;
            } else {
                st->active[k] = 0;
                if (deg >= 1) {
                    st->status = 7u;
                } else {
#pragma unroll
                    for (int i = 0; i < 8; i++) st->chan[i] = cs[i];
                    st->final_value = fv;
                    st->final_degree = deg;
                    st->chan_has = 1;
                    st->chan_pending = 0;
                }
            }
            s_beta_m = bm;
            s_active = active;
            s_deg = deg;
            TAIL_STAMP_T(15, 448, __builtin_amdgcn_s_memrealtime);
        }
        if (chan_wave) { has = 1; pending = 1; }
        lds_barrier();
        if (!s_active) break;
        beta_m = s_beta_m;
        prev_deg = s_deg;
    }
}

static LayerTask with_gate(const LayerTask& in) {
    LayerTask t = in;
    if (t.st) { t.gst = t.st; t.gidx = t.k > 0 ? t.k - 1 : -1; }
    return t;
}

#ifndef MID8
#define MID8 1
#endif
#ifndef QUAD_TPB
#define QUAD_TPB 512
#endif
#ifndef QUAD_MIN_LOG
#define QUAD_MIN_LOG 19
#endif

template <typename KernelLaunch>
static void pair_parts(LayerTask t, uint32_t G, hipStream_t s, const std::function<void()>& after_part1,
                       KernelLaunch&& go) {
    t.wg_total = G;
    if (!after_part1) {
        t.wg_base = 0;
        go(t, G);
        return;
    }
    const uint32_t h = G / 2;
    t.wg_base = t.send_half ? h : 0u;
    go(t, h);
    after_part1();
    t.wg_base = t.send_half ? 0u : h;
    go(t, h);
}

void launch_layer(const LayerTask& tin, hipStream_t s, hipEvent_t ev_leaf_end, const std::function<void()>& after_leaf,
                  hipEvent_t ev_before_top, const std::function<void()>& after_part1) {
    const LayerTask t = with_gate(tin);
    const uint32_t L = t.L;
    const bool fold = t.prev != nullptr;
    const bool commit = t.st != nullptr;
    const bool pair = t.prev2 != nullptr;
    const int32_t* nomx = nullptr;
    if (L <= TOP_LOG) {
        if (fold) {
            if (commit) hipLaunchKernelGGL((k_tree_top<true, true, true>), dim3(1), dim3(512), 0, s, t, 0u, nomx, 1u);
            else hipLaunchKernelGGL((k_tree_top<true, true, false>), dim3(1), dim3(512), 0, s, t, 0u, nomx, 1u);
        } else {
            if (commit) hipLaunchKernelGGL((k_tree_top<true, false, true>), dim3(1), dim3(512), 0, s, t, 0u, nomx, 1u);
            else hipLaunchKernelGGL((k_tree_top<true, false, false>), dim3(1), dim3(512), 0, s, t, 0u, nomx, 1u);
        }
        if (ev_leaf_end) hipEventRecord(ev_leaf_end, s);
        return;
    }
    uint32_t G, out_per_wg;
    if (L >= QUAD_MIN_LOG) {
        constexpr uint32_t TPB = QUAD_TPB;
        G = (uint32_t)(((size_t)1 << L) / (4 * TPB));
        out_per_wg = TPB / 4;
        if (pair) {
            pair_parts(t, G, s, after_part1, [&](const LayerTask& tp, uint32_t g) {
                hipLaunchKernelGGL((k_layer_leaf<true, false, TPB, true>), dim3(g), dim3(TPB), 0, s, tp);
            });
        } else if (fold) {
            if (commit) hipLaunchKernelGGL((k_layer_leaf<true, true, TPB>), dim3(G), dim3(TPB), 0, s, t);
            else hipLaunchKernelGGL((k_layer_leaf<true, false, TPB>), dim3(G), dim3(TPB), 0, s, t);
        } else {
            if (commit) hipLaunchKernelGGL((k_layer_leaf<false, true, TPB>), dim3(G), dim3(TPB), 0, s, t);
            else hipLaunchKernelGGL((k_layer_leaf<false, false, TPB>), dim3(G), dim3(TPB), 0, s, t);
        }
    } else {
        G = 1u << (L - 8);
        out_per_wg = 256u >> wide_levels(L);
        if (pair) {
            pair_parts(t, G, s, after_part1, [&](const LayerTask& tp, uint32_t g) {
                hipLaunchKernelGGL((k_layer_leaf_wide<true, false, true>), dim3(g), dim3(256), 0, s, tp);
            });
        } else if (fold) {
            if (commit) hipLaunchKernelGGL((k_layer_leaf_wide<true, true>), dim3(G), dim3(256), 0, s, t);
            else hipLaunchKernelGGL((k_layer_leaf_wide<true, false>), dim3(G), dim3(256), 0, s, t);
        } else {
            if (commit) hipLaunchKernelGGL((k_layer_leaf_wide<false, true>), dim3(G), dim3(256), 0, s, t);
            else hipLaunchKernelGGL((k_layer_leaf_wide<false, false>), dim3(G), dim3(256), 0, s, t);
        }
    }
    if (ev_leaf_end) hipEventRecord(ev_leaf_end, s);
    if (after_leaf) after_leaf();
    const int gate = t.gidx;
    const int32_t* mx = commit ? t.wgmax : nullptr;
    size_t mx_off = 3 * (size_t)G;
    uint32_t l = L >= QUAD_MIN_LOG ? 4u : wide_levels(L);
    while (L - l > TOP_LOG) {
        const size_t nodes = (size_t)1 << (L - l);
        const uint32_t nin = nodes >= ((size_t)1 << 18) ? 1024u : 256u;
        const uint32_t grid = (uint32_t)(nodes / nin);
        const uint32_t R = nin / out_per_wg;
        int32_t* mx_out = commit ? t.wgmax + mx_off : nullptr;
        const bool eight = nin == 256 && L - l >= 8 + 6 && MID8;
        if (nin == 1024)
            hipLaunchKernelGGL((k_tree_mid<1024>), dim3(grid), dim3(512), 0, s, t.tree, L, l, t.gst, gate, mx, mx_out, R);
        else if (eight)
            hipLaunchKernelGGL(k_tree_mid8, dim3(grid), dim3(256), 0, s, t.tree, L, l, t.gst, gate, mx, mx_out, R);
        else
            hipLaunchKernelGGL((k_tree_mid<256>), dim3(grid), dim3(128), 0, s, t.tree, L, l, t.gst, gate, mx, mx_out, R);
        if (commit) { mx = mx_out; mx_off += 3 * (size_t)grid; }
        G = grid;
        out_per_wg = eight ? 1u : nin / 16;
        l += eight ? 8u : 4u;
    }
    if (ev_before_top) hipStreamWaitEvent(s, ev_before_top, 0);
    if (commit) hipLaunchKernelGGL((k_tree_top<false, false, true>), dim3(1), dim3(512), 0, s, t, l, mx, G);
    else if (t.shard) hipLaunchKernelGGL((k_tree_top<false, false, false, true>), dim3(1), dim3(512), 0, s, t, l, nomx, G);
    else hipLaunchKernelGGL((k_tree_top<false, false, false>), dim3(1), dim3(512), 0, s, t, l, nomx, G);
}

void launch_tail(const LayerTask* ts, uint32_t n, hipStream_t s) {
    TailTask tt{};
    tt.n = n;
    for (uint32_t i = 0; i < n; i++) tt.t[i] = ts[i];
    tt.t[0] = with_gate(ts[0]);
    if (ts[0].prev) hipLaunchKernelGGL((k_tree_tail<true>), dim3(1), dim3(512), 0, s, tt);
    else hipLaunchKernelGGL((k_tree_tail<false>), dim3(1), dim3(512), 0, s, tt);
}

__global__ __launch_bounds__(256) void k_coef(LayerTask t) {
    if (gated_off(t)) return;
    __shared__ int32_t red[12];
    coef_task(t, blockIdx.x, gridDim.x, red);
}

void launch_coef(const LayerTask& tin, uint32_t G, hipStream_t s) {
    const LayerTask t = with_gate(tin);
    hipLaunchKernelGGL(k_coef, dim3(G), dim3(256), 0, s, t);
}

void launch_top(const LayerTask& tin, uint32_t l, const int32_t* mx, uint32_t G, hipStream_t s) {
    const LayerTask t = with_gate(tin);
    if (t.shard) hipLaunchKernelGGL((k_tree_top<false, false, true, true>), dim3(1), dim3(512), 0, s, t, l, mx, G);
    else hipLaunchKernelGGL((k_tree_top<false, false, true>), dim3(1), dim3(512), 0, s, t, l, mx, G);
}

}
```

Measured before the change: 3.670 billion field-elems/s.

## Fuse layer Merkle-top into next layer's fold kernel and write state to host directly

For small layers, the single-workgroup Merkle top kernel of layer k is deferred and merged into the next layer's fold/leaf kernel (k_layer_narrow) or into the tail kernel. Every workgroup redundantly recomputes the top hash chain to get beta, and only workgroup 0 stores the results. The channel state becomes per-layer (chan_lay) so redundant computation is safe, and wgmax buffers are double-buffered by layer parity. The final DevState copy-back memcpy is replaced by the tail kernel writing to mapped host memory. This removes serial single-block launches and a D2H copy, at the cost of redundant hashing per workgroup.

```diff
diff --git a/stark-prover_amd/csrc/fri_commit.hip b/stark-prover_amd/csrc/fri_commit.hip
--- a/stark-prover_amd/csrc/fri_commit.hip
+++ b/stark-prover_amd/csrc/fri_commit.hip
@@ -81,7 +81,7 @@
         dalloc(ctx, &p.trees, tre * 4) != hipSuccess || dalloc(ctx, &p.xinv, (xin ? xin : 1) * 4) != hipSuccess ||
         dalloc(ctx, &p.pre_lo, ((size_t)1 << POW_LO_LOG) * 4) != hipSuccess ||
         dalloc(ctx, &p.pre_hi, nhi * 4) != hipSuccess ||
-        dalloc(ctx, &p.wgmax, 6 * ((log_n > 8 ? ((size_t)1 << (log_n - 8)) : 1) + 16) * 4) != hipSuccess) {
+        dalloc(ctx, &p.wgmax, 2 * wgmax_half(log_n) * 4) != hipSuccess) {
         plan_release(ctx, p);
         return fail(ctx, FRI_ENOMEM, "device allocation failed for commit plan");
     }
@@ -108,6 +108,8 @@
     p.valid = true;
     return FRI_OK;
 }
+
+size_t fri::wgmax_half(uint32_t log_n) { return 6 * ((log_n > 8 ? ((size_t)1 << (log_n - 8)) : 1) + 16); }
 
 uint32_t* fri::coef_buf(Plan& p, int r) {
     if (r == 0) return const_cast<uint32_t*>(p.src);
@@ -126,12 +128,12 @@
     t.coef_in = coef_buf(p, k ? k - 1 : 0);
     t.coef_out = k ? coef_buf(p, k) : nullptr;
     t.d0 = p.d;
-    t.wgmax = p.wgmax;
+    t.wgmax = p.wgmax + (k & 1 ? wgmax_half(p.log_n) : 0);
     t.st = ctx->d_state;
     return t;
 }
 
-static void enqueue_commit(fri_ctx* ctx) {
+static void enqueue_commit(fri_ctx* ctx, DevState* hout) {
     Plan& p = ctx->plan;
     hipStream_t s = ctx->stream;
     const uint32_t log_n = p.log_n;
@@ -143,6 +145,7 @@
     size_t sp = span_begin(ctx, "lde", p.d * 4 + n * 4);
     launch_ntt(np, p.src, p.d, p.layers + p.layer_off[0], s);
     span_end(ctx, sp);
+    DeferredTop defer;
     for (int k = 0; k <= p.rmax; k++) {
         const uint32_t L = log_n - (uint32_t)k;
         if (L <= TAIL_LOG) {
@@ -150,17 +153,19 @@
             uint32_t nt = 0;
             for (int kk = k; kk <= p.rmax; kk++) ts[nt++] = commit_task(ctx, kk);
             size_t spk = span_begin(ctx, k == 0 ? "layer0" : "layers", 0);
-            launch_tail(ts, nt, s);
+            launch_tail(ts, nt, s, &defer, hout);
             span_end(ctx, spk);
             break;
         }
-        const LayerTask t = commit_task(ctx, k);
+        LayerTask t = commit_task(ctx, k);
+        if (k == p.rmax) t.hout = hout;
         uint64_t leaf_nodes = 0;
         for (uint32_t j = 0; j <= 4 && j <= L; j++) leaf_nodes += (uint64_t)1 << (L - j);
         const uint64_t leaf_bytes = ((uint64_t)4 << L) + 4 * (uint64_t)p.d + 32 * leaf_nodes;
         size_t spl = (k == 0 && L >= 19) ? span_begin(ctx, "merkle_layer0_leaf", leaf_bytes) : (size_t)-1;
         size_t spk = span_begin(ctx, k == 0 ? "layer0" : "layers", 0);
-        launch_layer(t, s, spl == (size_t)-1 ? nullptr : ctx->spans[spl].e);
+        defer.take = k < p.rmax && (narrow_merged(L - 1, k + 1) || (FRI_TAIL_TOP && L - 1 <= TAIL_LOG));
+        launch_layer(t, s, spl == (size_t)-1 ? nullptr : ctx->spans[spl].e, {}, nullptr, {}, &defer);
         span_end(ctx, spk);
     }
 }
@@ -221,6 +226,12 @@
             FRI_HIP(ctx, hipMemcpyAsync(p.d_in, dev_coeffs, d * 4, hipMemcpyDeviceToDevice, s));
         p.src = p.d_in;
     }
+    DevState* hs_dev = nullptr;
+    if (FRI_STATE_BY_KERNEL) {
+        void* dp = nullptr;
+        FRI_HIP(ctx, hipHostGetDevicePointer(&dp, hs, 0));
+        hs_dev = static_cast<DevState*>(dp);
+    }
     const bool use_graph = !(flags & FRI_FLAG_NO_GRAPH) && !ctx->profiling;
     if (use_graph) {
         const int gs = slot < 0 ? FRI_MAX_INFLIGHT : slot;
@@ -237,9 +248,10 @@
         if (!px) {
             FRI_HIP(ctx, hipStreamBeginCapture(s, hipStreamCaptureModeThreadLocal));
             hipError_t e1 = hipMemcpyAsync(ctx->d_state, hs, sizeof(DevState), hipMemcpyHostToDevice, s);
-            if (e1 == hipSuccess) enqueue_commit(ctx);
+            if (e1 == hipSuccess) enqueue_commit(ctx, hs_dev);
             const hipError_t e2 =
-                e1 == hipSuccess ? hipMemcpyAsync(hs, ctx->d_state, sizeof(DevState), hipMemcpyDeviceToHost, s) : e1;
+                e1 == hipSuccess && !hs_dev ? hipMemcpyAsync(hs, ctx->d_state, sizeof(DevState), hipMemcpyDeviceToHost, s)
+                                            : e1;
             hipGraph_t g = nullptr;
             const hipError_t e3 = hipStreamEndCapture(s, &g);
             if (e2 != hipSuccess || e3 != hipSuccess) {
@@ -254,9 +266,9 @@
         FRI_HIP(ctx, hipGraphLaunch(px, s));
     } else {
         FRI_HIP(ctx, hipMemcpyAsync(ctx->d_state, hs, sizeof(DevState), hipMemcpyHostToDevice, s));
-        enqueue_commit(ctx);
+        enqueue_commit(ctx, hs_dev);
         FRI_HIP(ctx, hipGetLastError());
-        FRI_HIP(ctx, hipMemcpyAsync(hs, ctx->d_state, sizeof(DevState), hipMemcpyDeviceToHost, s));
+        if (!hs_dev) FRI_HIP(ctx, hipMemcpyAsync(hs, ctx->d_state, sizeof(DevState), hipMemcpyDeviceToHost, s));
     }
     return FRI_OK;
 }
@@ -274,8 +286,8 @@
     out->final_degree = h->final_degree;
     for (uint32_t k = 0; k < h->n_layers && k <= (uint32_t)MAXR; k++) digest_to_bytes(h->roots[k], out->roots[k]);
     for (uint32_t r = 0; r < h->n_rounds && r < (uint32_t)MAXR; r++) out->betas[r] = h->beta[r];
-    digest_to_bytes(h->chan, out->channel_out.digest);
-    out->channel_out.has_state = h->chan_has;
+    digest_to_bytes(h->n_layers ? h->chan_lay[h->n_layers - 1] : h->chan, out->channel_out.digest);
+    out->channel_out.has_state = h->n_layers ? 1u : h->chan_has;
     ctx->err.clear();
     return FRI_OK;
 }
diff --git a/stark-prover_amd/csrc/fri_host.hpp b/stark-prover_amd/csrc/fri_host.hpp
--- a/stark-prover_amd/csrc/fri_host.hpp
+++ b/stark-prover_amd/csrc/fri_host.hpp
@@ -352,6 +352,7 @@
 int plan_build(fri_ctx* ctx, size_t d, uint32_t log_n, uint32_t offset, uint32_t G = 1, uint32_t rank = 0);
 uint32_t* coef_buf(Plan& p, int r);
 LayerTask commit_task(fri_ctx* ctx, int k);
+size_t wgmax_half(uint32_t log_n);
 void init_state(fri_ctx* ctx, DevState* h, const fri_channel_state* chan_in, uint32_t flags,
                 const uint32_t* forced_betas);
 int commit_validate(fri_ctx* ctx, size_t d, uint32_t log_n, uint32_t offset, uint32_t flags,
diff --git a/stark-prover_amd/csrc/fri_internal.hpp b/stark-prover_amd/csrc/fri_internal.hpp
--- a/stark-prover_amd/csrc/fri_internal.hpp
+++ b/stark-prover_amd/csrc/fri_internal.hpp
@@ -35,6 +35,7 @@
     uint32_t beta_mont[MAXR];
     uint32_t forced_beta[MAXR];
     uint32_t roots[MAXR + 1][8];
+    uint32_t chan_lay[MAXR + 1][8];
 #ifdef FRI_STAMPS
     uint64_t stamps[MAXR + 1][64];
 #endif
@@ -129,11 +130,36 @@
     uint32_t send_half;
     uint32_t wg_base;
     uint32_t wg_total;
+    DevState* hout;
+};
+#ifndef FRI_NARROW_MERGE
+#define FRI_NARROW_MERGE 1
+#endif
+#ifndef FRI_NARROW_MAX_LOG
+#define FRI_NARROW_MAX_LOG 16
+#endif
+#ifndef FRI_TAIL_TOP
+#define FRI_TAIL_TOP 1
+#endif
+#ifndef FRI_STATE_BY_KERNEL
+#define FRI_STATE_BY_KERNEL 1
+#endif
+inline bool narrow_merged(uint32_t L, int k) {
+    return FRI_NARROW_MERGE && k >= 1 && L > TAIL_LOG && L > TOP_LOG && L <= FRI_NARROW_MAX_LOG;
+}
+struct DeferredTop {
+    bool take = false;
+    bool pending = false;
+    LayerTask t;
+    uint32_t l = 0;
+    const int32_t* mx = nullptr;
+    uint32_t G = 0;
 };
 void launch_layer(const LayerTask& t, hipStream_t s, hipEvent_t ev_leaf_end = nullptr,
                   const std::function<void()>& after_leaf = {}, hipEvent_t ev_before_top = nullptr,
-                  const std::function<void()>& after_part1 = {});
-void launch_tail(const LayerTask* ts, uint32_t n, hipStream_t s);
+                  const std::function<void()>& after_part1 = {}, DeferredTop* defer = nullptr);
+void launch_tail(const LayerTask* ts, uint32_t n, hipStream_t s, DeferredTop* defer = nullptr,
+                 DevState* hout = nullptr);
 void launch_coef(const LayerTask& t, uint32_t G, hipStream_t s);
 void launch_coset_coeffs(const uint32_t* a, size_t d, uint32_t* out, size_t M, uint32_t c_std, hipStream_t s);
 void launch_decimate(const uint32_t* a, size_t d, uint32_t* ev, uint32_t* od, hipStream_t s);
diff --git a/stark-prover_amd/csrc/fri_layer.hip b/stark-prover_amd/csrc/fri_layer.hip
--- a/stark-prover_amd/csrc/fri_layer.hip
+++ b/stark-prover_amd/csrc/fri_layer.hip
@@ -9,15 +9,15 @@
 #ifdef FRI_STAMPS
 #define TOP_STAMP(i)                                                                     \
     do {                                                                                 \
-        if (COMMIT && threadIdx.x == 0) t.st->stamps[t.k][(i)] = __builtin_amdgcn_s_memrealtime(); \
+        if (COMMIT && blockIdx.x == 0 && threadIdx.x == 0) t.st->stamps[t.k][(i)] = __builtin_amdgcn_s_memrealtime(); \
     } while (0)
 #define TOP_CLK(i)                                                                               \
     do {                                                                                           \
-        if (COMMIT && threadIdx.x == 0) t.st->stamps[t.k][(i)] = __builtin_amdgcn_s_memtime();     \
+        if (COMMIT && blockIdx.x == 0 && threadIdx.x == 0) t.st->stamps[t.k][(i)] = __builtin_amdgcn_s_memtime();     \
     } while (0)
 #define TOP_STAMP_T(i, tid_)                                                                       \
     do {                                                                                           \
-        if (COMMIT && threadIdx.x == (tid_)) t.st->stamps[t.k][(i)] = __builtin_amdgcn_s_memrealtime(); \
+        if (COMMIT && blockIdx.x == 0 && threadIdx.x == (tid_)) t.st->stamps[t.k][(i)] = __builtin_amdgcn_s_memrealtime(); \
     } while (0)
 #else
 #define TOP_STAMP(i) do {} while (0)
@@ -93,7 +93,7 @@
     if (!real) return;
     const uint4 v = make_uint4(o[0], o[1], o[2], o[3]);
     B[2 * q + half] = v;
-    reinterpret_cast<uint4*>(out + 8 * q)[half] = v;
+    if (out) reinterpret_cast<uint4*>(out + 8 * q)[half] = v;
 }
 
 #ifndef FRI_SCHED_PRODUCER
@@ -135,7 +135,7 @@
     if (!real) return;
     const uint4 v = make_uint4(o[0], o[1], o[2], o[3]);
     B[2 * q + half] = v;
-    reinterpret_cast<uint4*>(out + 8 * q)[half] = v;
+    if (out) reinterpret_cast<uint4*>(out + 8 * q)[half] = v;
 }
 
 __device__ __forceinline__ void lds_barrier() {
@@ -149,7 +149,7 @@
 }
 
 __device__ __forceinline__ void coef_slice(const LayerTask& t, uint32_t w, uint32_t G, int32_t* red, uint32_t t0,
-                                           uint32_t nthr) {
+                                           uint32_t nthr, const uint32_t* prev = nullptr) {
     int m0 = -1, m1 = -1, m2 = -1;
     const uint32_t tx = threadIdx.x - t0;
     const size_t jhi_all = t.jhi ? t.jhi : ~(size_t)0;
@@ -164,8 +164,8 @@
         }
     } else {
         const DevState* st = t.st;
-        const size_t len = (size_t)(st->deg[t.k - 1] + 1), nlen = (len + 1) / 2;
-        const uint32_t beta_m = st->beta_mont[t.k - 1];
+        const size_t len = (size_t)((prev ? (int32_t)prev[0] : st->deg[t.k - 1]) + 1), nlen = (len + 1) / 2;
+        const uint32_t beta_m = prev ? prev[1] : st->beta_mont[t.k - 1];
         const size_t a = t.jlo, b = min(nlen, jhi_all), n = b > a ? b - a : 0;
         const size_t cs = (n + G - 1) / G, lo = a + (size_t)w * cs, hi = min(b, lo + cs);
         const uint32_t* in = t.coef_in - t.ibase;
@@ -545,14 +545,20 @@
     return add(add(add(t[0], t[1]), add(t[2], t[3])), add(add(t[4], t[5]), add(t[6], t[7])));
 }
 
-template <bool FROM_LEAVES, bool FOLD, bool COMMIT, bool SHARD = false>
-__global__ __launch_bounds__(512) void k_tree_top(LayerTask t, uint32_t l, const int32_t* mx, uint32_t G) {
-    if (gated_off(t)) return;
-    chain_prio();
-    __shared__ uint4 lds[2 * 1024 + 2 * 512];
-    __shared__ int32_t red[24];
-    __shared__ SchedLds sl;
-    sched_init(&sl);
+__device__ __forceinline__ void top_results(DevState* st, int k, int deg, const uint4* root_lds) {
+    st->deg[k] = deg;
+    Dg root;
+    dg_lds_load(root_lds, root);
+#pragma unroll
+    for (int i = 0; i < 8; i++) st->roots[k][i] = root.w[i];
+    st->n_layers = (uint32_t)k + 1;
+}
+
+enum { NEXT_DEG = 0, NEXT_BETA_M = 1, NEXT_ACTIVE = 2, NEXT_CHAN = 3, NEXT_WORDS = 11 };
+
+template <bool FROM_LEAVES, bool FOLD, bool COMMIT, bool SHARD>
+__device__ __forceinline__ void tree_top(const LayerTask& t, uint32_t l, const int32_t* mx, uint32_t G, uint4* Ain,
+                                         uint4* Bin, int32_t* red, SchedLds& sl, bool store, uint32_t* next) {
     const uint32_t L = t.L;
     const uint32_t N = 1u << (L - l);
     const uint32_t tid = threadIdx.x;
@@ -563,9 +569,10 @@
     uint32_t has = 0, forced = 0, fbeta = 0;
     int job = CJ_END_FINAL;
     if (chan_wave) {
-#pragma unroll
-        for (int i = 0; i < 8; i++) cs[i] = st->chan[i];
-        const uint32_t h = st->chan_has, pend = st->chan_pending;
+        const uint32_t* cin = t.k > 0 ? st->chan_lay[t.k - 1] : st->chan;
+#pragma unroll
+        for (int i = 0; i < 8; i++) cs[i] = cin[i];
+        const uint32_t h = t.k > 0 ? 1u : st->chan_has, pend = t.k > 0 ? 1u : st->chan_pending;
         const uint32_t fo = COMMIT ? st->forced : 0u, fb = st->forced_beta[t.k < MAXR ? t.k : 0];
         has = h;
         job = !h ? CJ_ROOT : (pend ? CJ_REHASH : CJ_MID);
@@ -573,8 +580,8 @@
         if (fo && t.k < MAXR) fbeta = fb;
     }
     if (tid >= 384 && tid < 448) kcache_touch_sha_tables();
-    uint4* A = lds;
-    uint4* B = lds + 2 * 1024;
+    uint4* A = Ain;
+    uint4* B = Bin;
     uint32_t* tr = t.tree;
     TOP_STAMP(0);
     if (FROM_LEAVES) {
@@ -669,7 +676,7 @@
         const bool level = it < nlev;
         if (level) {
             cnt >>= 1;
-            uint32_t* out = tr + 8 * level_offset(L, l + 1 + it);
+            uint32_t* out = store ? tr + 8 * level_offset(L, l + 1 + it) : nullptr;
             if (cnt <= 128) {
 #ifdef FRI_STAMPS
                 if (it < 18 && tid == 0) TOP_CLK(24 + 2 * it);
@@ -692,7 +699,7 @@
                     if (it < 18 && q == 0) TOP_CLK(25 + 2 * it);
 #endif
                     dg_lds_store(B + 2 * q, o);
-                    dg_store(out + 8 * q, o);
+                    if (store) dg_store(out + 8 * q, o);
                 }
             }
         }
@@ -731,51 +738,147 @@
     }
     if (!COMMIT || tid != 448) return;
     const int k = t.k;
+    uint32_t active = 0, bm = 0;
     if (noncanon) {
+        if (store) {
+            st->active[k] = 0;
+            st->status = 1u;
+        }
+    } else if (deg >= 1 && k < MAXR && L >= 1) {
+        uint32_t beta = chan_beta(cs);
+        if (forced) beta = fbeta;
+        bm = to_mont(beta);
+        active = 1;
+        if (store) {
+            top_results(st, k, deg, A);
+            TOP_STAMP_T(15, 448);
+#pragma unroll
+            for (int i = 0; i < 8; i++) st->chan_lay[k][i] = cs[i];
+            st->beta[k] = beta;
+            st->beta_mont[k] = bm;
+            st->active[k] = 1;
+            st->n_rounds = (uint32_t)k + 1;
+            TOP_STAMP_T(16, 448);
+        }
+    } else if (store) {
+        top_results(st, k, deg, A);
         st->active[k] = 0;
-        st->status = 1u;
-        return;
-    }
-    st->deg[k] = deg;
-    Dg root;
-    dg_lds_load(A, root);
-#pragma unroll
-    for (int i = 0; i < 8; i++) st->roots[k][i] = root.w[i];
-    st->n_layers = (uint32_t)k + 1;
-    TOP_STAMP_T(15, 448);
-    if (deg >= 1 && k < MAXR && L >= 1) {
-        uint32_t beta = chan_beta(cs);
-#pragma unroll
-        for (int i = 0; i < 8; i++) st->chan[i] = cs[i];
-        st->chan_has = 1;
-        st->chan_pending = 1;
-        if (forced) beta = fbeta;
-        st->beta[k] = beta;
-        st->beta_mont[k] = to_mont(beta);
-        st->active[k] = 1;
-        st->n_rounds = (uint32_t)k + 1;
-        TOP_STAMP_T(16, 448);
-    } else {
-        st->active[k] = 0;
-        if (deg >= 1) { st->status = 7u; return; }
-#pragma unroll
-        for (int i = 0; i < 8; i++) st->chan[i] = cs[i];
-        st->final_value = fv;
-        st->final_degree = deg;
-        st->chan_has = 1;
-        st->chan_pending = 0;
-    }
+        if (deg >= 1) {
+            st->status = 7u;
+        } else {
+#pragma unroll
+            for (int i = 0; i < 8; i++) st->chan_lay[k][i] = cs[i];
+            st->final_value = fv;
+            st->final_degree = deg;
+        }
+    }
+    if (next) {
+        next[NEXT_ACTIVE] = active;
+        next[NEXT_BETA_M] = bm;
+        next[NEXT_DEG] = (uint32_t)deg;
+#pragma unroll
+        for (int i = 0; i < 8; i++) next[NEXT_CHAN + i] = cs[i];
+    }
+}
+
+__device__ __forceinline__ void state_out(const DevState* st, DevState* hout) {
+    if (!hout) return;
+    __syncthreads();
+    const uint32_t* src = reinterpret_cast<const uint32_t*>(st);
+    uint32_t* dst = reinterpret_cast<uint32_t*>(hout);
+    for (uint32_t i = threadIdx.x; i < sizeof(DevState) / 4; i += blockDim.x) dst[i] = src[i];
+}
+
+template <bool FROM_LEAVES, bool FOLD, bool COMMIT, bool SHARD = false>
+__global__ __launch_bounds__(512) void k_tree_top(LayerTask t, uint32_t l, const int32_t* mx, uint32_t G) {
+    __shared__ uint4 lds[2 * 1024 + 2 * 512];
+    __shared__ int32_t red[24];
+    __shared__ SchedLds sl;
+    if (!gated_off(t)) {
+        chain_prio();
+        sched_init(&sl);
+        tree_top<FROM_LEAVES, FOLD, COMMIT, SHARD>(t, l, mx, G, lds, lds + 2 * 1024, red, sl, true, nullptr);
+    }
+    if (COMMIT) state_out(t.st, t.hout);
+}
+
+__global__ __launch_bounds__(512) void k_layer_narrow(LayerTask tp, uint32_t l, const int32_t* mx, uint32_t G,
+                                                      LayerTask t) {
+    if (gated_off(tp)) return;
+    __shared__ uint4 lds[2 * 512 + 2 * 256];
+    __shared__ int32_t red[24];
+    __shared__ SchedLds sl;
+    __shared__ uint32_t next[NEXT_WORDS];
+    [[maybe_unused]] constexpr bool COMMIT = true;
+    const uint32_t tid = threadIdx.x;
+    const uint32_t L = t.L;
+    const size_t wg = blockIdx.x, grid = gridDim.x;
+    const size_t i = wg * 256 + (tid & 255u);
+    uint32_t pa = 0, pb = 0, px = 0;
+    if (tid < 256) {
+        pa = t.prev[i];
+        pb = t.prev[i + ((size_t)1 << L)];
+        px = t.xinv[i];
+    }
+    chain_prio();
+    sched_init(&sl);
+    tree_top<false, false, true, false>(tp, l, mx, G, lds, lds + 2 * 512, red, sl, wg == 0, next);
+    lds_barrier();
+    if (!next[NEXT_ACTIVE]) return;
+    WIDE_STAMP(60);
+    const uint32_t beta_m = next[NEXT_BETA_M];
+    uint32_t* tr = t.tree;
+    uint4* A = lds;
+    uint4* B = lds + 2 * 256;
+    if (tid < 256) {
+        const uint32_t v = fold1(pa, pb, px, beta_m);
+        t.values[i] = v;
+        Dg d;
+        cleaf(v, d);
+        dg_store(tr + 8 * i, d);
+        dg_lds_store(A + 2 * tid, d);
+    }
+    lds_barrier();
+    WIDE_STAMP(61);
+    uint32_t cnt = 256;
+    const shaq::Role qr = shaq::role_of(tid);
+    const uint32_t nlev = wide_levels(L);
+    constexpr uint32_t ORD0 = 16;
+#pragma unroll 1
+    for (uint32_t j = 1; j <= nlev; j++) {
+        cnt >>= 1;
+        uint32_t* out = tr + 8 * (level_offset(L, j) + (wg << (8 - j)));
+        if ((size_t)cnt * grid < WIDE_PAIR_MAX) {
+            pair_level_s(A, B, out, tid, cnt, qr, &sl, ORD0 + j);
+        } else if (tid < cnt) {
+            Dg a, b, o;
+            dg_lds_load(A + 4 * tid, a);
+            dg_lds_load(A + 4 * tid + 2, b);
+            hnode(a, b, o);
+            dg_lds_store(B + 2 * tid, o);
+            dg_store(out + 8 * tid, o);
+        }
+        if (j == 2 && tid >= 128 && tid < 256) coef_slice(t, blockIdx.x, gridDim.x, red, 128, 128, next);
+        lds_barrier();
+        uint4* tmp = A; A = B; B = tmp;
+    }
+    if (tid == 128) coef_combine(t, blockIdx.x, red, 2);
+    WIDE_STAMP(62);
 }
 
 struct TailTask {
     LayerTask t[TAIL_LOG + 1];
     uint32_t n;
+    LayerTask top;
+    uint32_t top_l, top_G;
+    const int32_t* top_mx;
+    DevState* hout;
 };
 
-template <bool FOLD0>
-__global__ __launch_bounds__(512) void k_tree_tail(TailTask tt) {
+template <bool FOLD0, bool TOPA>
+__device__ __forceinline__ void tree_tail(const TailTask& tt) {
     const LayerTask& t0 = tt.t[0];
-    if (gated_off(t0)) return;
+    if (TOPA ? gated_off(tt.top) : gated_off(t0)) return;
     chain_prio();
     constexpr uint32_t NMAX = 1u << TAIL_LOG;
     __shared__ uint4 lds[2 * NMAX + NMAX];
@@ -802,19 +905,34 @@
     };
     uint32_t cs[8], X[4];
     uint32_t has = 0;
-    if (chan_wave) {
-#pragma unroll
-        for (int i = 0; i < 8; i++) cs[i] = st->chan[i];
-        has = st->chan_has;
-    }
-    uint32_t pending = chan_wave ? st->chan_pending : 0u;
-    if (tid >= 384 && tid < 448) kcache_touch_sha_tables();
+    uint32_t pending = 0;
+    __shared__ uint32_t next[NEXT_WORDS];
+    if (TOPA) {
+        tree_top<false, false, true, false>(tt.top, tt.top_l, tt.top_mx, tt.top_G, lds, lds + 2 * NMAX, red, sl, true,
+                                            next);
+        lds_barrier();
+        if (!next[NEXT_ACTIVE]) return;
+        ord = 16;
+        if (chan_wave) {
+#pragma unroll
+            for (int i = 0; i < 8; i++) cs[i] = next[NEXT_CHAN + i];
+            has = 1;
+            pending = 1;
+        }
+    } else if (chan_wave) {
+        const uint32_t* cin = t0.k > 0 ? st->chan_lay[t0.k - 1] : st->chan;
+#pragma unroll
+        for (int i = 0; i < 8; i++) cs[i] = cin[i];
+        has = t0.k > 0 ? 1u : st->chan_has;
+        pending = t0.k > 0 ? 1u : st->chan_pending;
+    }
+    if (!TOPA && tid >= 384 && tid < 448) kcache_touch_sha_tables();
     if (tid < tt.n + 1) {
         const int kk = t0.k + (int)tid;
         s_fbeta[tid] = (st->forced && kk < MAXR) ? st->forced_beta[kk] + 1u : 0u;
     }
-    uint32_t beta_m = FOLD0 ? st->beta_mont[t0.k - 1] : 0u;
-    int prev_deg = FOLD0 ? st->deg[t0.k - 1] : -1;
+    uint32_t beta_m = TOPA ? next[NEXT_BETA_M] : (FOLD0 ? st->beta_mont[t0.k - 1] : 0u);
+    int prev_deg = TOPA ? (int)next[NEXT_DEG] : (FOLD0 ? st->deg[t0.k - 1] : -1);
     const shaq::Role R = shaq::role_of(tid);
     uint32_t xoff = 0;
 #pragma unroll 1
@@ -963,9 +1081,7 @@
             if (deg >= 1 && k < MAXR && L >= 1) {
                 uint32_t beta = chan_beta(cs);
 #pragma unroll
-                for (int i = 0; i < 8; i++) st->chan[i] = cs[i];
-                st->chan_has = 1;
-                st->chan_pending = 1;
+                for (int i = 0; i < 8; i++) st->chan_lay[k][i] = cs[i];
                 if (s_fbeta[li]) beta = s_fbeta[li] - 1u;
                 st->beta[k] = beta;
                 bm = to_mont(beta);
@@ -979,11 +1095,9 @@
                     st->status = 7u;
                 } else {
 #pragma unroll
-                    for (int i = 0; i < 8; i++) st->chan[i] = cs[i];
+                    for (int i = 0; i < 8; i++) st->chan_lay[k][i] = cs[i];
                     st->final_value = fv;
                     st->final_degree = deg;
-                    st->chan_has = 1;
-                    st->chan_pending = 0;
                 }
             }
             s_beta_m = bm;
@@ -997,6 +1111,12 @@
         beta_m = s_beta_m;
         prev_deg = s_deg;
     }
+}
+
+template <bool FOLD0, bool TOPA = false>
+__global__ __launch_bounds__(512) void k_tree_tail(TailTask tt) {
+    tree_tail<FOLD0, TOPA>(tt);
+    state_out(tt.t[0].st, tt.hout);
 }
 
 static LayerTask with_gate(const LayerTask& in) {
@@ -1033,13 +1153,15 @@
 }
 
 void launch_layer(const LayerTask& tin, hipStream_t s, hipEvent_t ev_leaf_end, const std::function<void()>& after_leaf,
-                  hipEvent_t ev_before_top, const std::function<void()>& after_part1) {
+                  hipEvent_t ev_before_top, const std::function<void()>& after_part1, DeferredTop* defer) {
     const LayerTask t = with_gate(tin);
     const uint32_t L = t.L;
     const bool fold = t.prev != nullptr;
     const bool commit = t.st != nullptr;
     const bool pair = t.prev2 != nullptr;
     const int32_t* nomx = nullptr;
+    const bool narrow = defer && defer->pending;
+    if (narrow) defer->pending = false;
     if (L <= TOP_LOG) {
         if (fold) {
             if (commit) hipLaunchKernelGGL((k_tree_top<true, true, true>), dim3(1), dim3(512), 0, s, t, 0u, nomx, 1u);
@@ -1070,7 +1192,9 @@
     } else {
         G = 1u << (L - 8);
         out_per_wg = 256u >> wide_levels(L);
-        if (pair) {
+        if (narrow) {
+            hipLaunchKernelGGL(k_layer_narrow, dim3(G), dim3(512), 0, s, defer->t, defer->l, defer->mx, defer->G, t);
+        } else if (pair) {
             pair_parts(t, G, s, after_part1, [&](const LayerTask& tp, uint32_t g) {
                 hipLaunchKernelGGL((k_layer_leaf_wide<true, false, true>), dim3(g), dim3(256), 0, s, tp);
             });
@@ -1107,16 +1231,34 @@
         l += eight ? 8u : 4u;
     }
     if (ev_before_top) hipStreamWaitEvent(s, ev_before_top, 0);
+    if (commit && defer && defer->take) {
+        defer->pending = true;
+        defer->t = t;
+        defer->l = l;
+        defer->mx = mx;
+        defer->G = G;
+        return;
+    }
     if (commit) hipLaunchKernelGGL((k_tree_top<false, false, true>), dim3(1), dim3(512), 0, s, t, l, mx, G);
     else if (t.shard) hipLaunchKernelGGL((k_tree_top<false, false, false, true>), dim3(1), dim3(512), 0, s, t, l, nomx, G);
     else hipLaunchKernelGGL((k_tree_top<false, false, false>), dim3(1), dim3(512), 0, s, t, l, nomx, G);
 }
 
-void launch_tail(const LayerTask* ts, uint32_t n, hipStream_t s) {
+void launch_tail(const LayerTask* ts, uint32_t n, hipStream_t s, DeferredTop* defer, DevState* hout) {
     TailTask tt{};
     tt.n = n;
     for (uint32_t i = 0; i < n; i++) tt.t[i] = ts[i];
     tt.t[0] = with_gate(ts[0]);
+    tt.hout = hout;
+    if (defer && defer->pending) {
+        defer->pending = false;
+        tt.top = defer->t;
+        tt.top_l = defer->l;
+        tt.top_mx = defer->mx;
+        tt.top_G = defer->G;
+        hipLaunchKernelGGL((k_tree_tail<true, true>), dim3(1), dim3(512), 0, s, tt);
+        return;
+    }
     if (ts[0].prev) hipLaunchKernelGGL((k_tree_tail<true>), dim3(1), dim3(512), 0, s, tt);
     else hipLaunchKernelGGL((k_tree_tail<false>), dim3(1), dim3(512), 0, s, tt);
 }
```

Result: no change. 3.664 billion field-elems/s (-0.2%).
